# jizongFox/Self-paced-Contrastive-Learning

Hardware: AMD Instinct MI355X
Metric: pretrain slices/sec/node (UNet+InfoNCE, 224^2, bs=32/GPU) (higher is better)
Workload: dtype bf16; 1 GPU; BASELINE.json configs[1]: self-paced pretrain step, UNet base (max_channel=256) encoder to Conv5 + ProjectionHead(256,256,256) + SelfPacedSupConLoss(soft, partition labels, correct_grad) fwd+bwd + RAdam; slices_per_gpu=32, images_per_gpu_step=64, image=1x224x224, global_batch=32, parallelism=dp1, params=1311056, hipgraph=epocher, capture_steps=3

## Files before the change

include/spcl_hip.h:

```cpp
#ifndef SPCL_HIP_H
#define SPCL_HIP_H
#include <stddef.h>
#include <stdint.h>
#ifdef __cplusplus
extern "C" {
#endif

#define SPCL_F32 0
#define SPCL_BF16 1

#define SPCL_OK 0
#define SPCL_EINVAL (-1)
#define SPCL_ELAUNCH (-2)
#define SPCL_EUNSUPPORTED (-3)

#define SPCL_ABI_VERSION 18
int spcl_abi_version(void);
const char* spcl_last_error(void);

size_t spcl_supcon_workspace_bytes(int n, int d);
int spcl_supcon_forward(const float* z1, const float* z2, const float* labels, const float* mask, int n, int d,
                        float temperature, int sp_mode, float gamma, int correct_grad, float* ws, float* out,
                        void* stream);
int spcl_supcon_backward(const float* labels, const float* mask, int n, int d, float temperature, int sp_mode,
                         float gamma, const float* ws_fwd, float* ws_bwd, const float* out_fwd,
                         const float* grad_out, float* dz1, float* dz2, void* stream);
size_t spcl_supcon_bwd_workspace_bytes(int n, int d);
int spcl_supcon_unit_gradient_block(int n, int d, size_t* offset_floats, int* row_pitch);
int spcl_supcon_forward_heads(int K, const float* z1, const float* z2, size_t z_stride, const float* labels, int n,
                              int d, float temperature, int sp_mode, const float* gammas, int correct_grad, float* ws,
                              size_t ws_stride, float* out, void* stream);
int spcl_supcon_rows_supported(int n, int d);
int spcl_supcon_forward_rows(int K, const float* o1, const float* o2, size_t o_stride, const float* labels, int n, int d,
                             float temperature, int sp_mode, const float* gammas, int correct_grad, float* ws,
                             size_t ws_stride, float* out, void* stream);
int spcl_supcon_backward_heads(int K, const float* labels, int n, int d, float temperature, int sp_mode,
                               const float* gammas, const float* ws_fwd, size_t ws_stride, float* ws_bwd,
                               size_t wsb_stride, const float* out_fwd, const float* grad_out, float* dz1, float* dz2,
                               size_t z_stride, void* stream);
int spcl_supcon_materialize(const float* labels, const float* mask, int n, int d, float temperature, int sp_mode,
                            float gamma, const float* ws_fwd, float* sim_logits, float* sim_exp, float* pos_mask,
                            float* neg_mask, float* sp_mask, void* stream);

size_t spcl_supcon_xpos_workspace_bytes(int n, int d);
int spcl_supcon_xpos_forward(const float* z1, const float* z2, const float* labels, const float* mask, int n, int d,
                             float temperature, float* ws, float* out, void* stream);
int spcl_supcon_xpos_backward(const float* z1, const float* z2, int n, int d, float temperature, const float* ws,
                              const float* grad_out, float* dz1, float* dz2, void* stream);

// ... 28 lines not shown

int spcl_conv_pack_weights_block(const float* wa_oihw, int CinA, int CoutA, void* a_fwd, void* a_dgrad,
                                 const float* wb_oihw, int CinB, int CoutB, void* b_fwd, void* b_dgrad, int dtype,
                                 void* stream);
int spcl_conv_pack_weights_block_at(const float* wa_oihw, int CinA, int CoutA, void* a_fwd, void* a_dgrad,
                                    const float* wb_oihw, int CinB, int CoutB, void* b_fwd, void* b_dgrad, int dtype,
                                    int H, int W, void* stream);

#define SPCL_PACK_MULTI_MAX 24
typedef struct spcl_pack_item {
  const float* w_oihw;
  void* fwd;
  void* dgrad;
  int Cin, Cout, H, W;
} spcl_pack_item;
int spcl_conv_pack_weights_multi(const spcl_pack_item* items, int n, int dtype, void* stream);
int spcl_conv_pack_weights_multi_acorr(const spcl_pack_item* items, int n, int dtype, const float* image, int N, int H,
                                       int W, float* acorr, void* stream);
int spcl_conv_pack_weights_multi_zero(const spcl_pack_item* items, int n, int dtype, const float* image, int N, int H, int W,
                                      float* acorr, void* zero, size_t zero_bytes, void* stream);

int spcl_conv_num_tiles(int N, int H, int W);
int spcl_conv_stat_rows(int dtype, int N, int H, int W, int CinK, int CoutS);
void spcl_conv_set_gemm(int mode);
void spcl_conv_set_f32_split(int on);
int spcl_conv_get_f32_split(void);
size_t spcl_bn_stats_elems(int ntiles, int CS);
int spcl_conv3x3_forward(const void* x, int dtype, int N, int H, int W, int CinS, int CinK, int CoutS,
                         const void* w_packed, int in_mode, const float* in_scale, const float* in_shift, void* y,
                         float* stats, void* stream);
int spcl_conv3x3_forward_image_acorr_rows(int dtype, int N, int H, int W, int CinS, int CoutS);
int spcl_conv3x3_forward_image_acorr(const void* x, int dtype, int N, int H, int W, int CinS, int CoutS,
                                     const void* w_packed, void* y, float* stats, float* acorr_rows, void* stream);
int spcl_conv_cat_supported(int dtype, int N, int H, int W, int Chalf, int CoutS);
int spcl_conv3x3_forward_cat(const void* xa, const void* xb, int dtype, int N, int H, int W, int Chalf, int CoutS,
                             const void* w_packed, const float* xb_scale, const float* xb_shift, void* y, float* stats,
                             void* stream);
int spcl_conv3x3_wgrad_cat(const void* xa, const void* xb, const void* dy, int dtype, int N, int H, int W, int Chalf,
                           int Cout, int CoutS, const float* xb_scale, const float* xb_shift, float* partial,
                           float* dw_oihw, void* stream);
int spcl_conv_up2_supported(int dtype, int N, int H, int W, int CinK, int CoutS);
int spcl_conv3x3_forward_up2(const void* x_half, int dtype, int N, int H, int W, int CinK, int CoutS, const void* w_packed,
                             void* y, float* stats, void* stream);
int spcl_conv3x3_wgrad_up2(const void* x_half, const void* dy, int dtype, int N, int H, int W, int Cin, int Cout, int CoutS,
                           float* partial, float* dw_oihw, void* stream);
int spcl_conv_split_supported(int dtype, int N, int H, int W, int CinK, int CoutS);
int spcl_conv3x3_forward_split(const void* x, int dtype, int N, int H, int W, int CinK, int CoutS, const void* w_packed,
                               void* y_lo, void* y_hi, void* stream);
int spcl_conv_split_bnstats_supported(int dtype, int N, int H, int W, int CinK, int CoutS);
int spcl_conv3x3_dgrad_split_bnstats(const void* dy, int dtype, int N, int H, int W, int CinK, int CoutS,
                                     const void* w_packed, void* g_lo, void* g_hi, const void* y2_hi, const float* scale2,
                                     const float* shift2, const float* mean2, float* rows2, void* stream);

size_t spcl_conv_wgrad_workspace_bytes(int N, int H, int W, int CinK, int CoutS);
int spcl_conv3x3_wgrad(const void* x, const void* dy, int dtype, int N, int H, int W, int Cin, int CinS, int CinK,
                       int Cout, int CoutS, int in_mode, const float* in_scale, const float* in_shift, float* partial,
                       float* dw_oihw, void* stream);

int spcl_adaptive_pool2d_forward(const void* x, int dtype, int N, int H, int W, int C, int Cs, int OH, int OW, int mode,
                                 float* out, int* argmax, void* stream);
int spcl_adaptive_pool2d_backward(const float* dout, const int* argmax, int dtype, int N, int H, int W, int C, int Cs,
                                  int OH, int OW, int mode, void* dx, void* stream);

int spcl_l2norm_rows_forward(const float* x, size_t rows, int O, float* z, void* stream);
int spcl_l2norm_rows_backward(const float* x, const float* dz, size_t rows, int O, float* dx, void* stream);

// ... 57 lines not shown
                                      const float* scale, const float* shift, int training, float* ws, float* dgamma,
                                      float* dbeta, void* dy, void* stream);
int spcl_bnrelu_backward_up2(const void* y, const void* d_up, void* dact, int dtype, int N, int H, int W, int C, int CS,
                             const float* mean, const float* invstd, const float* scale, const float* shift, int training,
                             float* ws, float* dgamma, float* dbeta, void* dy, void* stream);
int spcl_bnrelu_backward_bcast(const void* y, const void* dact_nc, int dtype, int N, int H, int W, int C, int CS,
                               const float* mean, const float* invstd, const float* scale, const float* shift, int training,
                               float* ws, float* dgamma, float* dbeta, void* dy, void* stream);

size_t spcl_bnrelu_image_wgrad_workspace_bytes(int N, int H, int W, int CS);
int spcl_bnrelu_backward_image_wgrad(const void* y, const void* dact, const float* image, int dtype, int N, int H,
                                     int W, int C, int CS, const float* mean, const float* invstd, const float* scale,
                                     const float* shift, int training, float* ws, float* dgamma, float* dbeta,
                                     float* dw, void* stream);

int spcl_conv_dgrad_bnstats_supported(int dtype, int N, int H, int W, int CinK, int CoutS);
int spcl_conv3x3_dgrad_bnstats(const void* dy, int dtype, int N, int H, int W, int CinK, int CoutS, const void* w_packed,
                               void* g, const void* y2, const float* scale2, const float* shift2, const float* mean2,
                               float* rows2, void* stream);

int spcl_image_autocorr_rows(int N, int H, int W);
int spcl_image_autocorr(const float* image, int N, int H, int W, float* out, void* stream);
int spcl_conv_dgrad_bnstats_image_supported(int dtype, int N, int H, int W, int CinK, int CoutS);
int spcl_conv3x3_dgrad_bnstats_image(const void* dy, int dtype, int N, int H, int W, int CinK, int CoutS,
                                     const void* w_packed, void* g, const void* y2, const float* scale2,
                                     const float* shift2, const float* mean2, const float* image, float* rows11,
                                     void* stream);
int spcl_conv16_bwd_fused_supported(int dtype, int N, int H, int W, int CinK, int CoutS);
int spcl_conv16_bwd_fused_splits(int N, int H, int W);
int spcl_conv16_bwd_fused(const void* dy, int dtype, int N, int H, int W, const void* w_packed_dgrad, const void* y2,
                          const float* scale2, const float* shift2, const float* mean2, const float* image,
                          float* rows11, float* partial, float* dw_oihw, int Cin, int Cout, float* wg_rows,
                          const float* acorr, int nacorr, float* acorr16, void* stream);
int spcl_bnrelu_backward_wgrows_image3(const float* wg_rows, int nwg, const float* acorr, int nacorr, const float* w_oihw,
                                       int N, int H, int W, int C, int CS, const float* mean, const float* invstd,
                                       const float* scale, int training, float* ws, float* dgamma, float* dbeta,
                                       float* dw, void* stream);
size_t spcl_bnrelu_image3_workspace_bytes(int CS);
int spcl_bnrelu_backward_rows_image3(const float* rows11, int nrows, const float* acorr, int nacorr, const float* w_oihw,
                                     int N, int H, int W, int C, int CS, const float* mean, const float* invstd,
                                     const float* scale, int training, float* ws, float* dgamma, float* dbeta, float* dw,
                                     void* stream);

int spcl_conv_dgrad_poolstats_supported(int dtype, int N, int H, int W, int CinK, int CoutS, int H2, int W2);
int spcl_conv3x3_dgrad_poolstats(const void* dy, int dtype, int N, int H, int W, int CinK, int CoutS, const void* w_packed,
                                 void* g, const void* y2, int H2, int W2, const float* scale2, const float* shift2,
                                 const float* mean2, float* rows2, void* stream);
int spcl_bnrelu_pool_backward_rows(const void* y, const void* dpool, const float* rows, int nrows, int dtype, int N, int H,
                                   int W, int C, int CS, const float* mean, const float* invstd, const float* scale,
                                   const float* shift, int training, float* ws, float* dgamma, float* dbeta, void* dy,
                                   void* stream);
int spcl_bnrelu_backward_rows(const void* y, const void* dact, const float* image, const float* rows, int nrows, int dtype,
                              int N, int H, int W, int C, int CS, const float* mean, const float* invstd,
                              const float* scale, const float* shift, int training, float* ws, float* dgamma,
                              float* dbeta, void* dy, float* dw, void* stream);


int spcl_conv1x1_forward(const void* x, int dtype, size_t npix, int C, int CS, int K, const float* w, const float* b,
                         float* out, void* stream);
size_t spcl_conv1x1_bwd_workspace_bytes(int C, int K);
int spcl_conv1x1_backward(const void* x, const float* dout, int dtype, size_t npix, int C, int CS, int K, const float* w,
                          void* dx, float* dw, float* db, float* ws, void* stream);
int spcl_conv1x1_forward_bn(const void* y, int dtype, size_t npix, int C, int CS, int K, const float* scale,
                            const float* shift, const float* w, const float* b, float* out, void* stream);
int spcl_conv1x1_bwd_rows(size_t npix);
int spcl_conv1x1_backward_bn(const void* y, const float* dout, int dtype, size_t npix, int C, int CS, int K,
// ... 203 lines not shown
```

self-paced-contrastive-learning_amd/csrc/conv.hip:

```cpp
#include <stdlib.h>
#include "bn_acc.hpp"
#include "conv_common.hpp"
#include "image_acorr.hpp"

namespace spcl {

#ifndef SPCL_SPLIT_KC_MAX
#define SPCL_SPLIT_KC_MAX 64
#endif
__host__ __device__ inline int split_kc(int CinK, int CoutS) {
  const int cap = CoutS <= 16 ? 16 : (CoutS <= 32 ? 32 : SPCL_SPLIT_KC_MAX);
  return CinK < cap ? CinK : cap;
}
__host__ __device__ inline int split_pstride(int KC) {
  const int b = 3 * KC * 2;
  return (b / 32) % 2 == 1 ? b : b + 32;
}
__device__ __forceinline__ f32x4 mfma_bf16(u32x4 w, u32x4 x, f32x4 acc) {
  return __builtin_amdgcn_mfma_f32_16x16x32_bf16(__builtin_bit_cast(bf16x8, w), __builtin_bit_cast(bf16x8, x), acc, 0, 0, 0);
}

template <typename T, int TH, int TW, int NT, bool SPLIT = false>
__global__ __launch_bounds__(256) void conv3x3_mfma_kernel(ConvArgs a) {
  static_assert(!SPLIT || sizeof(T) == 4, "the split k-loop is the f32 storage path");
// ... 1062 lines not shown
  else if (dtype == SPCL_BF16) rc = launch_conv_t<bf16_t>(a, st);
  else {
    set_error("conv3x3_forward: dtype %d", dtype);
    return SPCL_EINVAL;
  }
  if (rc != 0) {
    set_error("conv3x3_forward: no kernel for N=%d H=%d W=%d CinK=%d CoutS=%d in_mode=%d", N, H, W, CinK, CoutS, in_mode);
    return SPCL_EUNSUPPORTED;
  }
  SPCL_LAUNCH_CHECK("conv3x3_forward");
  return SPCL_OK;
}

static bool image_acorr_args(ConvArgs& a, int dtype, int N, int H, int W, int CinS, int CoutS) {
  static const bool off = lab_env("SPCL_ACORR_IN_CONV", 1) == 0;
  if (off || dtype != SPCL_BF16 || N <= 0 || H <= 0 || W <= 0 || CinS != 1 || CoutS != 16) return false;
  a.N = N; a.H = H; a.W = W; a.CinS = CinS; a.CinK = 16; a.CoutS = CoutS; a.in_mode = 2;
  a.tilesX = a.tilesY = 0; a.tpw = 1; a.dbg = 0;
  const TileCfg t = pick_tile_k(H, W, 16, CoutS);
  static const int no_fast = lab_env("SPCL_CONV_NO_FAST", 0);
  return !no_fast && t.tw == 14 && t.th == 14 && H % 14 == 0 && W % 14 == 0;
}

extern "C" int spcl_conv3x3_forward_image_acorr_rows(int dtype, int N, int H, int W, int CinS, int CoutS) {
  ConvArgs a;
  float dummy = 0.f;
  a.x = nullptr; a.y = nullptr; a.wp = nullptr; a.stats = nullptr; a.in_scale = a.in_shift = nullptr;
  if (!image_acorr_args(a, dtype, N, H, W, CinS, CoutS)) return 0;
  a.acorr_rows = &dummy;
  if (!launch_conv_fast(a, 14, nullptr, true)) return 0;
  return N * cdiv(H, 14) * cdiv(W, 14);
}

extern "C" int spcl_conv3x3_forward_image_acorr(const void* x, int dtype, int N, int H, int W, int CinS, int CoutS,
                                                const void* w_packed, void* y, float* stats, float* acorr_rows,
                                                void* stream) {
  SPCL_CHECK_ARG(x && y && w_packed && acorr_rows, "conv3x3_forward_image_acorr: null pointer");
  ConvArgs a;
  a.x = x; a.y = y; a.wp = w_packed; a.stats = stats; a.in_scale = a.in_shift = nullptr;
  if (!image_acorr_args(a, dtype, N, H, W, CinS, CoutS)) {
    set_error("conv3x3_forward_image_acorr: unsupported configuration (ask spcl_conv3x3_forward_image_acorr_rows)");
    return SPCL_EUNSUPPORTED;
  }
  a.acorr_rows = acorr_rows;
  {
    const double px = (double)N * H * W;
    prof_cost(px * (4.0 + CoutS * 2.0) + 9.0 * 16 * CoutS * 2.0 + (double)N * cdiv(H, 14) * cdiv(W, 14) * 256.0,
              2.0 * px * 9.0 * CinS * CoutS + 2.0 * px * 2.0 * 256.0);
  }
  if (!launch_conv_fast(a, 14, (hipStream_t)stream)) {
    set_error("conv3x3_forward_image_acorr: no kernel for N=%d H=%d W=%d", N, H, W);
    return SPCL_EUNSUPPORTED;
  }
  SPCL_LAUNCH_CHECK("conv3x3_forward_image_acorr");
  return SPCL_OK;
}

static bool conv_cat_args(ConvArgs& a, int dtype, int N, int H, int W, int Chalf, int CoutS) {
  static const bool off = lab_env("SPCL_CONV_CAT", 1) == 0;
  if (off || dtype != SPCL_BF16 || N <= 0 || H <= 0 || W <= 0 || CoutS % 16 != 0 || CoutS <= 0 ||
      (Chalf != 16 && Chalf != 32 && Chalf != 64 && Chalf != 128))
    return false;
  if ((2 * Chalf) % 64 == 0 && CoutS % 64 == 0 && Chalf % 64 != 0) return false;
  a.in_scale = a.in_shift = nullptr;
  a.stats = nullptr;
  a.N = N; a.H = H; a.W = W; a.CinS = 2 * Chalf; a.CinK = 2 * Chalf; a.CoutS = CoutS; a.in_mode = 0;
  a.tilesX = a.tilesY = 0;
  a.tpw = 1;
  a.dbg = 0;
  return !conv_use_gemm(a.CinK, CoutS, H, W) && pick_tile(H, W).tw == 14;
}

extern "C" int spcl_conv_cat_supported(int dtype, int N, int H, int W, int Chalf, int CoutS) {
  ConvArgs a;
  if (!conv_cat_args(a, dtype, N, H, W, Chalf, CoutS)) return 0;
  static const char dummy[16] = {0};
  a.x = dummy; a.x2 = dummy; a.y = nullptr; a.wp = nullptr;
  return launch_conv_fast(a, pick_tile_k(H, W, a.CinK).th, nullptr, true) ? 1 : 0;
}

extern "C" int spcl_conv3x3_forward_cat(const void* xa, const void* xb, int dtype, int N, int H, int W, int Chalf, int CoutS,
                                        const void* w_packed, const float* xb_scale, const float* xb_shift, void* y,
                                        float* stats, void* stream) {
  SPCL_CHECK_ARG(xa && xb && y && w_packed, "conv3x3_forward_cat: null pointer");
  SPCL_CHECK_ARG((xb_scale == nullptr) == (xb_shift == nullptr), "conv3x3_forward_cat: xb_scale and xb_shift come together");
  SPCL_CHECK_ARG(xb_scale == nullptr || Chalf <= 32, "conv3x3_forward_cat: the raw second tensor exists for Chalf 16 / 32 only");
  SPCL_CHECK_ARG((uintptr_t)xa % 16 == 0 && (uintptr_t)xb % 16 == 0, "conv3x3_forward_cat: inputs must be 16-byte aligned");
// ... 343 lines not shown
```

self-paced-contrastive-learning_amd/csrc/conv16_bwd.hip:

```cpp
#include <stdio.h>
#include <stdlib.h>
#include <vector>
#include "conv_common.hpp"

namespace spcl {

struct Bwd16Args {
  const unsigned char* dy;
  const u32x4* wp;
  const unsigned char* y2;
  const float* scale2;
  const float* shift2;
  const float* mean2;
  const float* img;
  float* rows11;
  float* wg_rows;
  int nwg;
  const float* acorr_in;
  int nacorr;
  float* acorr_out;
  float* partial;
  int N, H, W, tilesX, tilesY, ipw, xcd_remap;
  int dbg;
  unsigned long long* stamps;
};

constexpr int B16_TH = 14, B16_TW = 14, B16_HW = 16, B16_RP = 22, B16_PS = 32;
constexpr int B16_DY = 0, B16_DY_BYTES = (B16_TH + 2) * B16_RP * B16_PS;
constexpr int B16_IM = B16_DY_BYTES, B16_IM_BYTES = 1536;
constexpr int B16_XT = B16_IM + B16_IM_BYTES, B16_XT_ROW = 16 * 32, B16_XT_BYTES = B16_TH * B16_XT_ROW;
constexpr int B16_RED = B16_XT + B16_XT_BYTES;
constexpr int B16_ACC = B16_RED + 512;
constexpr int B16_TRASH = B16_ACC + 576;
constexpr int B16_LDS = B16_TRASH + 32;

#ifndef SPCL_CONV16_DBG_BUILD
#define SPCL_CONV16_DBG_BUILD 0
#endif
#define B16_DBG(a) (SPCL_CONV16_DBG_BUILD ? (a).dbg : 0)

__device__ __forceinline__ bf16x8 b16_tr_frag(unsigned addr) {
  const s16x4 lo = __builtin_amdgcn_ds_read_tr16_b64_v4i16((s16x4 __attribute__((address_space(3)))*)(uintptr_t)addr);
  const s16x4 hi =
// ... 360 lines not shown
        for (int w = 1; w < NW; ++w) tot += red[32 * w];
      } else {
        tot = ((const float*)(lds + B16_ACC))[i - 32];
      }
      a.wg_rows[(size_t)i * a.nwg + wg] = tot;
    }
  }
  float* out = a.partial + wg * (9 * 256);
#pragma unroll
  for (int j = 0; j < TPW; ++j) {
    const int tap = wave + NW * j;
    if (tap < 9) {
#pragma unroll
      for (int r = 0; r < 4; ++r) out[(tap * 16 + 4 * ((t0 & 63) >> 4) + r) * 16 + (t0 & 15)] = wacc[j][r];
    }
  }
}


#ifndef SPCL_CONV16_ROWS_WPE
#define SPCL_CONV16_ROWS_WPE 4
#endif
constexpr int r16_wpe(bool shifted) { return shifted && SPCL_CONV16_ROWS_WPE > 3 ? 3 : SPCL_CONV16_ROWS_WPE; }
constexpr int R16_RP = 18;
constexpr int R16_DY = 0, R16_DY_BYTES = (B16_TH + 2) * R16_RP * B16_PS;
constexpr int R16_IM = R16_DY_BYTES;
constexpr int R16_XT = R16_IM + B16_IM_BYTES;
constexpr int R16_RED = R16_XT + B16_XT_BYTES;
constexpr int R16_ACC = R16_RED + 512;
constexpr int R16_TRASH = R16_ACC + 576;
constexpr int R16_TAB = R16_TRASH + 32;
constexpr int B16_LDS_ROWS = R16_TAB + 128;

template <bool SHIFTED, bool WGROWS>
__global__ __launch_bounds__(128) __attribute__((amdgpu_waves_per_eu(r16_wpe(SHIFTED)))) void conv16_bwd_rows_kernel(Bwd16Args a) {
  constexpr int NW = 2;
  constexpr int TH = B16_TH, TW = B16_TW, HW_ = B16_HW, RP = R16_RP, PS = B16_PS;
  constexpr int NSTEPS = 5, NTHR = 64 * NW, ITER = 512 / NTHR, RPI = NTHR / 32;
  constexpr int MW = TH / NW, TPW = (9 + NW - 1) / NW;
  static_assert(TH % NW == 0, "rows are dealt to the waves evenly");
  extern __shared__ __attribute__((aligned(16))) unsigned char lds[];
  const unsigned lds_base = (unsigned)(uintptr_t)(unsigned char __attribute__((address_space(3)))*)lds;
  const int t0 = threadIdx.x;
  const int wave = __builtin_amdgcn_readfirstlane(t0 >> 6);
  if (WGROWS && (int)blockIdx.z * (int)(gridDim.x * gridDim.y) >= a.nwg) {
    const int nslice = gridDim.x * gridDim.y;
    float* fold = (float*)lds;
    const int cq = t0 & 15, rl = t0 >> 4;
    for (int j = blockIdx.y * gridDim.x + blockIdx.x; j < 16; j += nslice) {
      f32x4 sacc = {0.f, 0.f, 0.f, 0.f};
#pragma unroll 16
      for (int w = j + 16 * rl; w < a.nacorr; w += 128) sacc += *(const f32x4*)(a.acorr_in + (size_t)w * 64 + 4 * cq);
      __syncthreads();
      *(f32x4*)(fold + rl * 64 + 4 * cq) = sacc;
      __syncthreads();
      if (t0 < 64) {
        float tot = fold[t0];
#pragma unroll
        for (int r = 1; r < 8; ++r) tot += fold[r * 64 + t0];
        a.acorr_out[(size_t)j * 64 + t0] = tot;
      }
    }
    return;
  }

  int tx = blockIdx.x, ty = blockIdx.y;
  {
    const int T = a.tilesX * a.tilesY;
// ... 1 lines not shown
      const int L = ty * a.tilesX + tx;
      const int L2 = (L & 7) * (T >> 3) + (L >> 3);
      ty = L2 / a.tilesX;
      tx = L2 - ty * a.tilesX;
    }
  }
  const int y0 = min(ty * TH, a.H - TH), x0 = min(tx * TW, a.W - TW);
  const int oy = ty * TH - y0, ox = tx * TW - x0;
  const bool interior = y0 > 0 && x0 > 0 && y0 + TH < a.H && x0 + TW < a.W;
  const bool shifted = SHIFTED && (oy | ox) != 0;

  if (t0 < 4 * TH) *(u32x4*)(lds + R16_XT + (t0 >> 2) * B16_XT_ROW + TW * PS + (t0 & 3) * 16) = (u32x4){0u, 0u, 0u, 0u};
  if (t0 >= NTHR - 64)
    *(u32x4*)(lds + R16_DY + (((t0 & 63) >> 2) * RP + HW_) * PS + (t0 & 3) * 16) = (u32x4){0u, 0u, 0u, 0u};
  if (t0 < 48) {
    const int r = t0 & 15, k = t0 >> 4;
    ((bf16_t*)(lds + R16_IM))[(k == 0 ? 256 + 15 : (k == 1 ? 512 + 14 : 512 + 15)) + r * 16] = 0;
  }
  if (t0 >= 64 && t0 < 64 + 20) {
    const int e = t0 - 64, gq = e / NSTEPS, s = e - gq * NSTEPS;
    int fc = 4 * s + gq;
    if (fc >= 18) fc = 0;
    const int tap = fc >> 1, c = fc & 1, ky = (tap * 11) >> 5, kx = tap - 3 * ky;
    ((unsigned*)(lds + R16_TAB))[gq * 8 + s] = (unsigned)((ky * RP + kx) * PS + c * 16);
  }
  if (WGROWS)
    for (int i = t0; i < (512 + 576) / 4; i += NTHR) ((float*)(lds + R16_RED))[i] = 0.f;
  f32x4 wacc[TPW];
#pragma unroll
  for (int j = 0; j < TPW; ++j) wacc[j] = (f32x4){0.f, 0.f, 0.f, 0.f};

  float imgv[256 / NTHR];
  u32x4 v[ITER];
  uint2 ypre[MW];
  constexpr int PPT = 256 / NTHR;
  auto rsrc = [](const void* p) { return __builtin_amdgcn_make_buffer_rsrc((void*)p, 0, 0x7fffffff, 0x00020000); };
  constexpr int OOB = (int)0x80000000u;
  auto issue_img = [&](const int n) {
    int t = t0;
    asm volatile("" : "+v"(t));
    const int hr = (t * PPT) >> 4, hc = (t * PPT) & 15;
    const int gy = y0 - 1 + hr;
    const __amdgpu_buffer_rsrc_t rs = rsrc(a.img + (size_t)n * a.H * a.W);
    const int rowo = (gy < 0 ? 0 : (gy >= a.H ? a.H - 1 : gy)) * a.W;
#pragma unroll
    for (int e = 0; e < PPT; ++e) {
      const int gx = x0 - 1 + hc + e;
      imgv[e] = __builtin_bit_cast(float, __builtin_amdgcn_raw_buffer_load_b32(rs, (rowo + (gx < 0 ? 0 : (gx >= a.W ? a.W - 1 : gx))) * 4, 0, 0));
    }
  };
  auto issue_halo = [&](const int n) {
    int t = t0;
    asm volatile("" : "+v"(t));
    const int ch = t & 1, q0 = t >> 1, hy0 = q0 / HW_, hx0 = q0 % HW_;
    const int voff = (hy0 * a.W + hx0) * 32 + ch * 16;
    const __amdgpu_buffer_rsrc_t rs = rsrc(a.dy + (((long)n * a.H + (y0 - 1)) * a.W + (x0 - 1)) * 32);
#pragma unroll
    for (int k = 0; k < ITER; ++k) {
      bool inb = true;
      if (!interior) {
        const int gy = y0 - 1 + hy0 + RPI * k, gx = x0 - 1 + hx0;
        inb = gy >= 0 && gy < a.H && gx >= 0 && gx < a.W;
      }
      v[k] = __builtin_bit_cast(u32x4, __builtin_amdgcn_raw_buffer_load_b128(rs, inb ? voff : OOB, RPI * k * a.W * 32, 0));
    }
  };
  auto issue_y2 = [&](const int n) {
    int t = t0;
    asm volatile("" : "+v"(t));
    const int r16 = t & 15, g = (t & 63) >> 4;
    const int voff = min(r16, TW - 1) * 32 + g * 8;
    const __amdgpu_buffer_rsrc_t rs = rsrc(a.y2 + (((size_t)n * a.H + y0 + wave) * a.W + x0) * 32);
#pragma unroll
    for (int j = 0; j < MW; ++j)
      ypre[j] = __builtin_bit_cast(uint2, __builtin_amdgcn_raw_buffer_load_b64(rs, voff, NW * j * a.W * 32, 0));
  };
  const __amdgpu_buffer_rsrc_t rs_wp = rsrc(a.wp), rs_sc = rsrc(a.scale2), rs_sh = rsrc(a.shift2), rs_mu = rsrc(a.mean2);

  const bool stamp = SPCL_CONV16_STAMPS_BUILD && a.stamps != nullptr && t0 == 0;
  unsigned long long tph[7] = {0, 0, 0, 0, 0, 0, 0}, tc = 0;
  const int n_first = blockIdx.z * a.ipw;
  if (stamp) tc = __builtin_amdgcn_s_memtime();
  if (n_first < a.N) {
    issue_img(n_first);
    issue_halo(n_first);
    issue_y2(n_first);
  }
  __syncthreads();
  uint2 dzp[MW];
  auto second_half = [&](const int n) {
    int t = t0;
    asm volatile("" : "+v"(t));
    const int lane = t & 63, r16 = t & 15, g = lane >> 4;
    const int tile = (n * a.tilesY + ty) * a.tilesX + tx;
    const unsigned xaddr = (unsigned)(R16_XT + wave * B16_XT_ROW + r16 * PS + (((g + (r16 >> 2)) & 3) << 3));
    B16_STAMP(3)
    __syncthreads();
    B16_STAMP(1)
    if (!WGROWS && t < 32) {
      const float* red = (const float*)(lds + R16_RED) + t;
      float tot = red[0];
#pragma unroll
      for (int w = 1; w < NW; ++w) tot += red[32 * w];
      a.rows11[(size_t)tile * 11 * 16 + t] = tot;
    }

    const unsigned tr_col = (unsigned)((4 * (g & 1) + (r16 >> 2)) * PS + (r16 & 3) * 8);
    const unsigned tr_x = lds_base + R16_XT + (g >> 1) * B16_XT_ROW + (4 * (g & 1) + (r16 >> 2)) * PS + ((((r16 & 3) + (g & 1)) & 3) << 3);
    const unsigned tr_xh = (tr_x + 8 * PS) ^ 16u;
    {
      unsigned ad[TPW];
#pragma unroll
      for (int j = 0; j < TPW; ++j) {
        const int tap = min(wave + NW * j, 8), ky = tap / 3, kx = tap - 3 * ky;
        ad[j] = lds_base + R16_DY + (g >> 1) * RP * PS + tr_col + (2 - ky) * RP * PS + (2 - kx) * PS;
      }
#pragma unroll
      for (int ks = 0; ks < TH / 2; ++ks) {
        const bf16x8 af = b16_tr_frag2(tr_x + ks * 2 * B16_XT_ROW, tr_xh + ks * 2 * B16_XT_ROW);
// ... 49 lines not shown
    const f32x4 mu2 = __builtin_bit_cast(f32x4, __builtin_amdgcn_raw_buffer_load_b128(rs_mu, g * 16, 0, 0));
    if (r16 >= TW || (SHIFTED && r16 < ox)) {
      sc2 = (f32x4){0.f, 0.f, 0.f, 0.f};
      sh2 = (f32x4){-1.f, -1.f, -1.f, -1.f};
    }
    const u32x4 tabA = *(const u32x4*)(lds + R16_TAB + g * 32);
    const unsigned tabB = *(const unsigned*)(lds + R16_TAB + g * 32 + 16);
    {
      const int hr = (t * PPT) >> 4, hc = (t * PPT) & 15;
      const int gy = y0 - 1 + hr;
#pragma unroll
      for (int e = 0; e < PPT; ++e) {
        const int gx = x0 - 1 + hc + e;
        const float hv = (interior || (gy >= 0 && gy < a.H && gx >= 0 && gx < a.W)) ? imgv[e] : 0.f;
        const bf16_t hb = f32_to_bf16(hv);
        bf16_t* imb = (bf16_t*)(lds + R16_IM) + hr * 16 + hc + e;
        imb[0] = hb;
        if (hc + e >= 1) imb[256 - 1] = hb;
        if (hc + e >= 2) imb[512 - 2] = hb;
      }
    }
    {
      const int ch = t & 1, q0 = t >> 1, hy0 = q0 / HW_, hx0 = q0 % HW_;
      unsigned char* const lp = lds + R16_DY + (hy0 * RP + hx0) * PS + ch * 16;
#pragma unroll
      for (int k = 0; k < ITER; ++k) *(u32x4*)(lp + (RPI * k * RP) * PS) = v[k];
    }
    B16_STAMP(0)
    __syncthreads();
    B16_STAMP(1)

    f32x4 ssum = {0.f, 0.f, 0.f, 0.f}, ssq = {0.f, 0.f, 0.f, 0.f};
    const unsigned xaddr = (unsigned)(R16_XT + wave * B16_XT_ROW + r16 * PS + (((g + (r16 >> 2)) & 3) << 3));
    {
      const unsigned lb = (unsigned)(R16_DY + (wave * RP + r16) * PS);
      const unsigned offs[NSTEPS] = {tabA[0] + lb, tabA[1] + lb, tabA[2] + lb, tabA[3] + lb, tabB + lb};
#pragma unroll
      for (int j = 0; j < MW; ++j) {
        f32x4 acc = {0.f, 0.f, 0.f, 0.f};
#pragma unroll
        for (int s = 0; s < NSTEPS; ++s) {
          const u32x4 xf = *(const u32x4*)(lds + offs[s] + j * (NW * RP * PS));
          acc = mfma_chunk<bf16_t>(wall[s], xf, acc);
        }
        const bool keep_y = !shifted || wave + NW * j >= oy;
        const float yv[4] = {__uint_as_float(ypre[j].x << 16), __uint_as_float(ypre[j].x & 0xffff0000u),
                             __uint_as_float(ypre[j].y << 16), __uint_as_float(ypre[j].y & 0xffff0000u)};
        const f32x2 glo = {acc[0], acc[1]}, ghi = {acc[2], acc[3]};
        const uint32_t g0 = __builtin_bit_cast(uint32_t, __builtin_convertvector(glo, bf16x2v));
        const uint32_t g1 = __builtin_bit_cast(uint32_t, __builtin_convertvector(ghi, bf16x2v));
        const float gv[4] = {__uint_as_float(g0 << 16), __uint_as_float(g0 & 0xffff0000u),
                             __uint_as_float(g1 << 16), __uint_as_float(g1 & 0xffff0000u)};
        float xv[4], dz[4];
#pragma unroll
        for (int r = 0; r < 4; ++r) {
          float z = fmaf(sc2[r], yv[r], sh2[r]);
          if (SHIFTED) z = keep_y ? z : -1.f;
          xv[r] = z;
          dz[r] = z > 0.f ? gv[r] : 0.f;
          ssum[r] += dz[r];
          ssq[r] = fmaf(dz[r], yv[r] - mu2[r], ssq[r]);
        }
        const f32x2 lo = {xv[0], xv[1]}, hi = {xv[2], xv[3]};
        uint2 w;
        w.x = relu_bf16x2(__builtin_bit_cast(uint32_t, __builtin_convertvector(lo, bf16x2v)));
        w.y = relu_bf16x2(__builtin_bit_cast(uint32_t, __builtin_convertvector(hi, bf16x2v)));
        *(uint2*)(lds + xaddr + j * (NW * B16_XT_ROW)) = w;
        dzp[j].x = (__float_as_uint(dz[0]) >> 16) | (__float_as_uint(dz[1]) & 0xffff0000u);
        dzp[j].y = (__float_as_uint(dz[2]) >> 16) | (__float_as_uint(dz[3]) & 0xffff0000u);
        asm volatile("" : "+v"(dzp[j].x), "+v"(dzp[j].y));
        __builtin_amdgcn_sched_barrier(0);
      }
    }
    B16_STAMP(2)
    {
      f32x4 o;
#pragma unroll
      for (int r = 0; r < 4; ++r) {
        const float s1 = row16_sum(ssum[r]), s2 = row16_sum(ssq[r]);
        o[r] = r16 == 0 ? s1 : s2;
      }
      if (r16 < 2) {
        f32x4* rp = (f32x4*)(lds + R16_RED + ((wave * 2 + r16) * 16 + 4 * g) * 4);
        *rp = WGROWS ? *rp + o : o;
      }
    }
    if (!(it + 1 < a.ipw && n + 1 < a.N)) break;
    issue_halo(n + 1);
    issue_y2(n + 1);
    issue_img(n + 1);
    second_half(n);
  }
  if (n_first < a.N) second_half(n);

  if (stamp) {
    unsigned long long* o = a.stamps + ((size_t)(blockIdx.z * gridDim.y + blockIdx.y) * gridDim.x + blockIdx.x) * 8;
#pragma unroll
    for (int k = 0; k < 7; ++k) o[k] = tph[k];
  }
  const size_t wg = (size_t)(blockIdx.z * gridDim.y + blockIdx.y) * gridDim.x + blockIdx.x;
  if (WGROWS) {
    __syncthreads();
    for (int i = t0; i < 11 * 16; i += NTHR) {
      float tot;
      if (i < 32) {
        const float* red = (const float*)(lds + R16_RED) + i;
        tot = red[0];
#pragma unroll
        for (int w = 1; w < NW; ++w) tot += red[32 * w];
      } else {
        tot = ((const float*)(lds + R16_ACC))[i - 32];
      }
      a.wg_rows[(size_t)i * a.nwg + wg] = tot;
    }
  }
  float* out = a.partial + wg * (9 * 256);
#pragma unroll
  for (int j = 0; j < TPW; ++j) {
    const int tap = wave + NW * j;
    if (tap < 9) {
#pragma unroll
      for (int r = 0; r < 4; ++r) out[(tap * 16 + 4 * ((t0 & 63) >> 4) + r) * 16 + (t0 & 15)] = wacc[j][r];
// ... 8 lines not shown

int conv16_bwd_nw() {
  static const int env = lab_env("SPCL_CONV16_NW", 2);
  return env == 1 || env == 4 ? env : 2;
}

int conv16_bwd_ipw(int N, int H, int W) {
  const int nw = conv16_bwd_nw();
  const int resident = 256 * (nw == 1 ? 8 : (nw == 2 ? (conv16_bwd_rowmap() ? 2 * SPCL_CONV16_ROWS_WPE : 6) : 3));
  const long tiles = (long)cdiv(H, B16_TH) * cdiv(W, B16_TW);
  static const int env_ipw = lab_env("SPCL_CONV16_IPW", 0);
  int ipw = env_ipw > 0 ? env_ipw : (int)((tiles * N + resident - 1) / resident);
  if (ipw < 1) ipw = 1;
  if (ipw > N) ipw = N;
  return ipw;
}

}

using namespace spcl;

extern "C" int spcl_conv16_bwd_fused_supported(int dtype, int N, int H, int W, int CinK, int CoutS) {
  static const bool off = lab_flag("SPCL_NO_CONV16_FUSED");
  if (off || CinK != 16 || CoutS != 16) return 0;
  return spcl_conv_dgrad_bnstats_image_supported(dtype, N, H, W, CinK, CoutS);
}

extern "C" int spcl_conv16_bwd_fused_splits(int N, int H, int W) {
  if (N <= 0 || H < B16_TH || W < B16_TW) return 0;
  const int ipw = conv16_bwd_ipw(N, H, W);
  return cdiv(H, B16_TH) * cdiv(W, B16_TW) * cdiv(N, ipw);
}

extern "C" int spcl_conv16_bwd_fused(const void* dy, int dtype, int N, int H, int W, const void* w_packed_dgrad,
                                     const void* y2, const float* scale2, const float* shift2, const float* mean2,
                                     const float* image, float* rows11, float* partial, float* dw_oihw, int Cin, int Cout,
                                     float* wg_rows, const float* acorr, int nacorr, float* acorr16, void* stream) {
  SPCL_CHECK_ARG(dy && w_packed_dgrad && y2 && scale2 && shift2 && mean2 && image && partial && dw_oihw,
                 "conv16_bwd_fused: null pointer");
  SPCL_CHECK_ARG((rows11 != nullptr) != (wg_rows != nullptr), "conv16_bwd_fused: exactly one of rows11 / wg_rows");
  SPCL_CHECK_ARG(wg_rows == nullptr || (acorr && acorr16 && nacorr > 0), "conv16_bwd_fused: wg_rows comes with the autocorrelation rows");
  SPCL_CHECK_ARG(Cin > 0 && Cin <= 16 && Cout > 0 && Cout <= 16, "conv16_bwd_fused: channel counts");
  if (!spcl_conv16_bwd_fused_supported(dtype, N, H, W, 16, 16)) {
    set_error("conv16_bwd_fused: unsupported configuration (bf16, 16 -> 16 channels, 14 x 14 tiles)");
    return SPCL_EUNSUPPORTED;
  }
  hipStream_t st = (hipStream_t)stream;
  spcl_wgrad_tail* tail = take_tail_capture();
  Bwd16Args a;
  a.dy = (const unsigned char*)dy; a.wp = (const u32x4*)w_packed_dgrad; a.y2 = (const unsigned char*)y2;
  a.scale2 = scale2; a.shift2 = shift2; a.mean2 = mean2; a.img = image; a.rows11 = rows11; a.partial = partial;
  a.wg_rows = wg_rows; a.acorr_in = acorr; a.nacorr = nacorr; a.acorr_out = acorr16;
  a.N = N; a.H = H; a.W = W; a.tilesX = cdiv(W, B16_TW); a.tilesY = cdiv(H, B16_TH);
  a.ipw = conv16_bwd_ipw(N, H, W);
  static const int env_remap = lab_env("SPCL_CONV_XCD_REMAP", 1);
  a.xcd_remap = env_remap;
  a.dbg = lab_env("SPCL_CONV16_DBG", 0);
  const int nz = cdiv(N, a.ipw), nsplit = a.tilesX * a.tilesY * nz;
  a.nwg = nsplit;
  const double px = (double)N * H * W;
  prof_cost(px * 32.0 * 2.0 + px * 4.0 + (double)nsplit * 9 * 256 * 4.0, 2.0 * px * 9.0 * 256 * 2.0 + 2.0 * px * 9.0 * 16);
  a.stamps = nullptr;
  const bool want_stamps = SPCL_CONV16_STAMPS_BUILD && lab_flag("SPCL_CONV16_STAMPS");
  const size_t nwg = (size_t)nsplit;
  if (want_stamps) {
    (void)hipMalloc(&a.stamps, nwg * 8 * sizeof(unsigned long long));
    (void)hipMemset(a.stamps, 0, nwg * 8 * sizeof(unsigned long long));
  }
  const int nw = conv16_bwd_nw();
  const bool even = H % B16_TH == 0 && W % B16_TW == 0, wgr = wg_rows != nullptr;
  const dim3 grid(a.tilesX, a.tilesY, nz + (wgr ? 1 : 0));
#define B16_LAUNCH(SH_, NW_, WG_) SPCL_LAUNCH((conv16_bwd_kernel<SH_, NW_, WG_>), grid, dim3(64 * NW_), B16_LDS, st, a)
#define B16_CASE(NW_)                                       \
  if (nw == NW_) {                                          \
    if (even && wgr) B16_LAUNCH(false, NW_, true);          \
    else if (even) B16_LAUNCH(false, NW_, false);           \
    else if (wgr) B16_LAUNCH(true, NW_, true);              \
    else B16_LAUNCH(true, NW_, false);                      \
  }
  if (nw == 2 && conv16_bwd_rowmap()) {
#define B16_ROWS(SH_, WG_) SPCL_LAUNCH((conv16_bwd_rows_kernel<SH_, WG_>), grid, dim3(128), B16_LDS_ROWS, st, a)
    if (even && wgr) B16_ROWS(false, true);
    else if (even) B16_ROWS(false, false);
    else if (wgr) B16_ROWS(true, true);
    else B16_ROWS(true, false);
#undef B16_ROWS
  }
#if SPCL_LAB
  else {
    B16_CASE(1) B16_CASE(2) B16_CASE(4)
  }
#endif
#undef B16_CASE
#undef B16_LAUNCH
  if (a.stamps != nullptr) {
    std::vector<unsigned long long> h(nwg * 8);
    (void)hipStreamSynchronize(st);
    (void)hipMemcpy(h.data(), a.stamps, h.size() * 8, hipMemcpyDeviceToHost);
    (void)hipFree(a.stamps);
    double ph[7] = {0, 0, 0, 0, 0, 0, 0};
    for (size_t i = 0; i < nwg; ++i)
      for (int k = 0; k < 7; ++k) ph[k] += (double)h[i * 8 + k];
    fprintf(stderr, "[conv16_bwd stamps] %zu workgroups x %d tiles | s_memtime ticks of wave 0 per TILE: staging %.0f, barriers %.0f, "
            "dgrad %.0f, pixel pass %.0f, wgrad %.0f, dz stores %.0f, tap sums %.0f\n", nwg, a.ipw, ph[0] / nwg / a.ipw,
            ph[1] / nwg / a.ipw, ph[2] / nwg / a.ipw, ph[3] / nwg / a.ipw, ph[4] / nwg / a.ipw, ph[5] / nwg / a.ipw,
            ph[6] / nwg / a.ipw);
  }
  if (tail != nullptr) {
    tail->partial = partial; tail->dw = dw_oihw; tail->kind = 0; tail->nsplit = nsplit; tail->nblk_ci = 1;
    tail->nblk_co = 1; tail->CIB = 16; tail->COB = 16; tail->Cin = Cin; tail->Cout = Cout;
  } else {
    launch_wgrad_reduce(partial, nsplit, 1, 1, 16, 16, Cin, Cout, dw_oihw, st);
  }
  SPCL_LAUNCH_CHECK("conv16_bwd_fused");
  return SPCL_OK;
}
```

self-paced-contrastive-learning_amd/csrc/conv_common.hpp:

```cpp
#pragma once
#include "common.hpp"

namespace spcl {

struct BnAccFwd;
template <typename T> struct Chunk;
template <> struct Chunk<float> { static constexpr int EPC = 4; };
template <> struct Chunk<bf16_t> { static constexpr int EPC = 8; };

struct uint4_ { uint32_t x, y, z, w; };
typedef __attribute__((ext_vector_type(4))) uint32_t u32x4;

__host__ __device__ inline int conv_kc(int CinK) { return CinK < 64 ? CinK : 64; }
template <typename T> __host__ __device__ inline int conv_pstride(int KC) {
  int b = KC * (int)sizeof(T);
  return b == 32 ? 32 : b + 32;
}
template <typename T> __host__ __device__ inline int conv_nsteps(int KC) {
  int cp = KC / Chunk<T>::EPC;
  return (9 * cp + 3) / 4;
}

struct ConvArgs {
  const void* x;
  void* y;
  const void* wp;
  float* stats;
  const float* in_scale;
  const float* in_shift;
  int N, H, W;
  int CinS;
  int CinK;
  int CoutS;
  int in_mode;
  int tilesX, tilesY;
  int tpw;
  int dbg;
  const void* y2 = nullptr;
  const float* scale2 = nullptr;
  const float* shift2 = nullptr;
  const float* mean2 = nullptr;
  float* rows2 = nullptr;
  int H2 = 0, W2 = 0;
  const float* img2 = nullptr;
  const void* x2 = nullptr;
  void* y_hi = nullptr;
  bool x_up2 = false;
  float* acorr_rows = nullptr;
  long long* stats_acc = nullptr;
  long long* rows2_acc = nullptr;
  const struct BnAccFwd* in_bn = nullptr;
};

struct split_f32 { float v; };
template <> struct Chunk<split_f32> { static constexpr int EPC = 4; };
bool conv_f32_split();

typedef __attribute__((ext_vector_type(2))) float f32x2_;
typedef __attribute__((ext_vector_type(2))) __bf16 bf16x2v_;
struct Split3 { uint32_t hi, mid, lo; };
__device__ __forceinline__ Split3 split3_pair(float v0, float v1) {
  Split3 o;
  f32x2_ v = {v0, v1};
  o.hi = __builtin_bit_cast(uint32_t, __builtin_convertvector(v, bf16x2v_));
  v[0] -= __uint_as_float(o.hi << 16);
  v[1] -= __uint_as_float(o.hi & 0xffff0000u);
  o.mid = __builtin_bit_cast(uint32_t, __builtin_convertvector(v, bf16x2v_));
  v[0] -= __uint_as_float(o.mid << 16);
  v[1] -= __uint_as_float(o.mid & 0xffff0000u);
  o.lo = __builtin_bit_cast(uint32_t, __builtin_convertvector(v, bf16x2v_));
  return o;
}
__device__ __forceinline__ void split3_chunk(const float* e, u32x4& ph, u32x4& pm, u32x4& pl) {
#pragma unroll
  for (int k = 0; k < 4; ++k) {
    const Split3 o = split3_pair(e[2 * k], e[2 * k + 1]);
    ph[k] = o.hi;
    pm[k] = o.mid;
    pl[k] = o.lo;
  }
}
// ... 90 lines not shown
```

self-paced-contrastive-learning_amd/csrc/conv_fast.hip:

```cpp
#include <stdlib.h>
#include <type_traits>
#include <vector>
#include "bn_acc.hpp"
#include "conv_common.hpp"

namespace spcl {

struct FastArgs {
  const unsigned char* x;
  const unsigned char* x2;
  unsigned char* y;
  unsigned char* y_hi;
  int up2;
  const u32x4* wp;
  float* stats;
  const float* in_scale;
  const float* in_shift;
  int N, H, W, CinK, CoutS, tilesX, tilesY, gy;
  unsigned long long* stamps;
  int lds_flip;
  int xcd_remap;
  const unsigned char* y2;
  const float* scale2;
  const float* shift2;
  const float* mean2;
  float* rows2;
  int H2, W2;
  const float* img2;
  float* acorr_rows;
  long long* stats_acc;
  long long* rows2_acc;
  BnAccFwd in_bn;
};

#ifndef SPCL_FAST_WPE_NT1
#define SPCL_FAST_WPE_NT1 2
#endif
#ifndef SPCL_FAST_WPE_NT1_NW4
#define SPCL_FAST_WPE_NT1_NW4 3
#endif
#ifndef SPCL_FAST_WR_NT1
#define SPCL_FAST_WR_NT1 9
#endif
#ifndef SPCL_FAST_WPE_KC32
#define SPCL_FAST_WPE_KC32 2
#endif
#ifndef SPCL_FAST_YPRE_MINKC
#define SPCL_FAST_YPRE_MINKC 16
#endif
#ifndef SPCL_FAST_WIDE_STORES
#define SPCL_FAST_WIDE_STORES 1
#endif
#ifndef SPCL_FAST_DBG
#define SPCL_FAST_DBG 0
#endif
#ifndef SPCL_FAST_ROWMAP
#define SPCL_FAST_ROWMAP 1
#endif
#ifndef SPCL_FAST_RP
#define SPCL_FAST_RP (SPCL_FAST_ROWMAP ? 18 : 22)
#endif
#ifndef SPCL_FAST_RP_NARROW
#define SPCL_FAST_RP_NARROW (SPCL_FAST_ROWMAP ? 18 : 22)
#endif
constexpr int fast_pixel_stride(int KC) { return KC == 16 ? 32 : KC * 2 + 32; }
constexpr int fast_row_pitch(int KC) { return KC == 64 ? SPCL_FAST_RP : SPCL_FAST_RP_NARROW; }
constexpr int fast_lds_bytes(int KC, int TH) { return (TH + 2) * fast_row_pitch(KC) * fast_pixel_stride(KC); }
constexpr bool fast_preload_slab(int KC, int NW, int NT) { return KC == 32 || (KC == 64 && NW >= 2 && NT >= 1); }
constexpr int fast_wpe(int KC, int TH, int NW, int NT, int MODE = 0) {
  const int wgs = 160 * 1024 / fast_lds_bytes(KC, TH);
  int w = (wgs * NW + 3) / 4;
  w = w > 4 ? 4 : (w < 1 ? 1 : w);
  const int acc = (SPCL_FAST_ROWMAP ? TH : (TH * 14 + 15) / 16) * NT * 4;
  if (KC == 16 && MODE >= 2 && SPCL_FAST_YPRE_MINKC <= 16 && w > 3 && acc <= 80) return 3;
  if (acc > 80 && w > 2) return 2;
  if (KC == 64 && NT == 1 && NW == 4 && w > 2) return SPCL_FAST_WPE_NT1_NW4;
  if (KC == 64 && NT == 1 && NW >= 2 && w > 2) return SPCL_FAST_WPE_NT1;
  if (KC == 32 && fast_preload_slab(KC, NW, NT) && w > SPCL_FAST_WPE_KC32) return SPCL_FAST_WPE_KC32;
  if (fast_preload_slab(KC, NW, NT) && w > 2) return 2;
  return w;
}

template <int KC, int TH, int NT, int MODE, int NW>
__global__ __launch_bounds__(64 * NW) __attribute__((amdgpu_waves_per_eu(fast_wpe(KC, TH, NW, NT, MODE)))) void
conv3x3_fast_kernel(FastArgs a) {
  constexpr int TW = 14, HW_ = 16, CP = KC / 8, NHALO = (TH + 2) * HW_, PS = fast_pixel_stride(KC);
  constexpr int RP = fast_row_pitch(KC);
  constexpr int NTHR = 64 * NW, NCH = NHALO * CP, ITER = (NCH + NTHR - 1) / NTHR, QS = NTHR / CP;
  constexpr bool RM = SPCL_FAST_ROWMAP != 0;
  constexpr int NPIX = TH * TW, MT = RM ? TH : (NPIX + 15) / 16, NSTEPS = (9 * CP + 3) / 4;
  constexpr bool PRELOAD_W = KC == 16;
  constexpr bool PRELOAD_SLAB = fast_preload_slab(KC, NW, NT);
  static_assert(QS >= HW_ ? QS % HW_ == 0 : HW_ % QS == 0, "staging walk needs whole/even halo rows per iteration");
  extern __shared__ __attribute__((aligned(16))) unsigned char lds[];

  const int t = threadIdx.x, lane = t & 63, wave = t >> 6, r16 = lane & 15, g = lane >> 4;
#ifndef SPCL_FAST_STAMPS_BUILD
#define SPCL_FAST_STAMPS_BUILD 0
#endif
  const bool stamp = SPCL_FAST_STAMPS_BUILD && a.stamps != nullptr && t == 0;
  unsigned long long t_begin = 0, t_k0 = 0, t_k1 = 0, t_store = 0;
  if (stamp) t_begin = __builtin_amdgcn_s_memtime();
  int tx = blockIdx.x, ty = blockIdx.y;
  {
    const int T = a.tilesX * a.tilesY;
    if (a.xcd_remap && (T & 7) == 0) {
      const int L = ty * a.tilesX + tx;
      const int L2 = (L & 7) * (T >> 3) + (L >> 3);
      ty = L2 / a.tilesX;
      tx = L2 - ty * a.tilesX;
    }
  }
  int n = blockIdx.z, by = 0;
#if SPCL_FAST_DBG & 4
  if (KC == 64 && a.CinK >= 128 && gridDim.z == 2u * a.N * a.gy) n >>= 1;
#endif
  if (a.gy > 1) {
    by = n / a.N;
    n -= by * a.N;
  }
  const int y0 = min(ty * TH, a.H - TH), x0 = min(tx * TW, a.W - TW);
  const int oy = ty * TH - y0, ox = tx * TW - x0;
  const int tile = (n * a.tilesY + ty) * a.tilesX + tx;
  const int ntn = a.CoutS >> 4;
  const int nt0 = (by * NW + wave) * NT;
  const bool interior = y0 > 0 && x0 > 0 && y0 + TH < a.H && x0 + TW < a.W;
#if SPCL_FAST_DBG & 4
  const int nslab = KC < 64 ? 1 : ((a.CinK >= 128 && gridDim.z == 2u * a.N * a.gy) ? a.CinK / KC / 2 : a.CinK / KC);
#else
  const int nslab = KC < 64 ? 1 : a.CinK / KC;
#endif
  const int gps = (KC < 64 ? KC : a.CinK) * 2;

  constexpr bool M2 = MODE == 2 || MODE == 4;
  constexpr bool M1 = MODE == 1 || MODE >= 5;
  constexpr int ACC_TPC = MODE == 5 ? 4 : (MODE == 6 ? 2 : 1);
  float imgv[MODE == 4 ? 4 : 1];
  if (MODE == 4) {
    const int hr = lane >> 2, hc = (lane & 3) * 4;
    const int gy = y0 - 1 + hr;
    const float* ir = a.img2 + ((size_t)n * a.H + (gy < 0 ? 0 : (gy >= a.H ? a.H - 1 : gy))) * a.W;
#pragma unroll
    for (int e = 0; e < 4; ++e) {
      const int gx = x0 - 1 + hc + e;
      const bool in = gy >= 0 && gy < a.H && gx >= 0 && gx < a.W;
      const float xv = ir[gx < 0 ? 0 : (gx >= a.W ? a.W - 1 : gx)];
      imgv[e] = in ? xv : 0.f;
    }
  }

  u32x4 wall[PRELOAD_W ? NSTEPS : 1][NT];
  if (PRELOAD_W) {
#pragma unroll
    for (int s = 0; s < NSTEPS; ++s)
#pragma unroll
      for (int j = 0; j < NT; ++j) wall[s][j] = a.wp[(size_t)(s * ntn + nt0 + j) * 64 + lane];
  }

  const int ch = t & (CP - 1), q0 = t / CP;
  const int hy0 = q0 / HW_, hx0 = q0 % HW_;
  const bool two = a.x2 != nullptr;
  const bool two_chunks = two && a.CinK == KC;
  const int gps1 = two ? gps / 2 : gps;
  const int ch1 = two_chunks ? (ch & (CP / 2 - 1)) : ch;
  const long xorg = (((long)n * a.H + (y0 - 1)) * a.W + (x0 - 1)) * gps1;
  const unsigned char* xb = ((two_chunks && ch >= CP / 2) ? a.x2 : a.x) + xorg;
  const unsigned char* xb2 = two ? a.x2 + xorg : nullptr;
  const unsigned voff = (unsigned)((hy0 * a.W + hx0) * gps1 + ch1 * 16);
  unsigned char* const lp = lds + (hy0 * RP + hx0) * PS + ch * 16;

  int abase[MT];
#pragma unroll
  for (int i = 0; i < MT; ++i) {
    if (RM) {
      abase[i] = (i * RP + r16) * PS + (CP >= 4 ? g * 16 : 0);
    } else {
      int p = 16 * i + r16;
      if (p >= NPIX) p = 0;
      const int py = p / TW, px = p - py * TW;
      abase[i] = (py * RP + px) * PS + (CP >= 4 ? g * 16 : 0);
    }
  }
  f32x4 acc[MT][NT];
#pragma unroll
  for (int i = 0; i < MT; ++i)
#pragma unroll
    for (int j = 0; j < NT; ++j) acc[i][j] = (f32x4){0.f, 0.f, 0.f, 0.f};

  const int flip = a.lds_flip;
  const unsigned wvo = (unsigned)(nt0 * 64 + lane) * 16u;
  const size_t wstep = (size_t)ntn * 1024;
  u32x4 v[ITER];
  float ssc[8], ssh[8];
  constexpr bool STREAM_W = PRELOAD_SLAB && KC == 64;
  constexpr int WR = STREAM_W ? (NT == 1 ? SPCL_FAST_WR_NT1 : 9) : (PRELOAD_SLAB ? NSTEPS : 1);
  u32x4 wsl[WR][NT];
  constexpr bool acc_in = MODE >= 5;
  float* const coef_l = (float*)(lds + fast_lds_bytes(KC, TH) * (a.lds_flip != 0 ? 2 : 1));
  auto load_coef_lds = [&](int slab) {
    const int cc = two_chunks ? ch1 : ch;
#pragma unroll
    for (int e = 0; e < 8; e += 4) {
      *(f32x4*)&ssc[e] = *(const f32x4*)(coef_l + slab * KC + cc * 8 + e);
      *(f32x4*)&ssh[e] = *(const f32x4*)(coef_l + a.CinK + slab * KC + cc * 8 + e);
    }
  };
  auto issue_halo = [&](int slab, const bool first = false) {
    if (acc_in) {
      if (!first) load_coef_lds(slab);
    } else if (M1) {
#pragma unroll
      for (int e = 0; e < 8; e += 4) {
        const int cc = two_chunks ? ch1 : ch;
        *(f32x4*)&ssc[e] = *(const f32x4*)(a.in_scale + slab * KC + cc * 8 + e);
        *(f32x4*)&ssh[e] = *(const f32x4*)(a.in_shift + slab * KC + cc * 8 + e);
      }
    }
    const int hslab = (a.CinK / KC) >> 1;
    const unsigned char* xs = (two && !two_chunks) ? (slab >= hslab ? xb2 + (slab - hslab) * (KC * 2) : xb + slab * (KC * 2))
                                                   : xb + slab * (KC * 2);
    auto walk = [&](auto up2_c, auto interior_c) {
      constexpr bool UP2 = decltype(up2_c)::value, INTERIOR = decltype(interior_c)::value;
#pragma unroll
      for (int k = 0; k < ITER; ++k) {
        const int dky = QS >= HW_ ? k * (QS / HW_) : k / (HW_ / QS);
        const int dkx = QS >= HW_ ? 0 : (k % (HW_ / QS)) * QS;
        const long soff = ((long)dky * a.W + dkx) * gps1;
        bool inb = (NCH % NTHR == 0) || (k * NTHR + t < NCH);
        if (!INTERIOR) {
          const int gy = y0 - 1 + hy0 + dky, gx = x0 - 1 + hx0 + dkx;
// ... 3 lines not shown
        if (UP2) {
          const int gy = y0 - 1 + hy0 + dky, gx = x0 - 1 + hx0 + dkx;
          if (inb)
            v[k] = *(const u32x4*)(a.x + (((long)n * (a.H >> 1) + (gy >> 1)) * (a.W >> 1) + (gx >> 1)) * gps + slab * (KC * 2) +
                                   ch * 16);
        } else if (inb) v[k] = *(const u32x4*)(xs + soff + voff);
      }
    };
    if (a.up2) walk(std::true_type{}, std::false_type{});
    else if (interior) walk(std::false_type{}, std::true_type{});
    else walk(std::false_type{}, std::false_type{});
  };
  unsigned char* lpw = lp;
  auto slab_body = [&](const int slab, const bool refill) {
    auto stage = [&](auto interior_c) {
      constexpr bool INTERIOR = decltype(interior_c)::value;
#pragma unroll
      for (int k = 0; k < ITER; ++k) {
        const int dky = QS >= HW_ ? k * (QS / HW_) : k / (HW_ / QS);
        const int dkx = QS >= HW_ ? 0 : (k % (HW_ / QS)) * QS;
        const bool in_range = (NCH % NTHR == 0) || (k * NTHR + t < NCH);
        u32x4 tv = v[k];
        if (M1) {
          bool inb = true;
          if (!INTERIOR) {
            const int gy = y0 - 1 + hy0 + dky, gx = x0 - 1 + hx0 + dkx;
            inb = gy >= 0 && gy < a.H && gx >= 0 && gx < a.W;
          }
          if (inb && (!two_chunks || ch >= CP / 2)) tv = bnrelu_regs<bf16_t>(tv, ssc, ssh);
        }
        if (in_range) *(u32x4*)(lpw + (dky * RP + dkx) * PS) = tv;
      }
    };
    if (M1 && !interior) stage(std::false_type{});
    else stage(std::true_type{});
    if (refill) issue_halo(slab + 1);
    if (stamp && slab == 0) t_store = __builtin_amdgcn_s_memtime();
    __syncthreads();
    if (stamp && slab == 0) t_k0 = __builtin_amdgcn_s_memtime();

    const u32x4* wslab = a.wp + ((size_t)slab * NSTEPS * ntn + nt0) * 64 + lane;
    auto frag_off = [&](const int s) {
      if (CP >= 4) {
        const int fc0 = 4 * s, tap = fc0 / CP, c0 = fc0 % CP, ky = tap / 3, kx = tap % 3;
        return (ky * RP + kx) * PS + c0 * 16;
      }
      int fc = 4 * s + g;
      if (fc >= 9 * CP) fc = 0;
      const int tap = fc / CP, c = fc % CP, ky = (tap * 11) >> 5, kx = tap - 3 * ky;
      return (ky * RP + kx) * PS + c * 16;
    };
    if (STREAM_W) {
      const __amdgpu_buffer_rsrc_t wrs = __builtin_amdgcn_make_buffer_rsrc((void*)a.wp, 0, 0x7fffffff, 0x00020000);
      unsigned wrun = (unsigned)(((size_t)slab * NSTEPS + WR) * wstep);
      u32x4 xf[2][MT];
#pragma unroll
      for (int i = 0; i < MT; ++i) xf[0][i] = *(const u32x4*)(lds + abase[i] + frag_off(0));
#pragma unroll
      for (int s = 0; s < NSTEPS; ++s) {
        u32x4 wf[NT];
#pragma unroll
        for (int j = 0; j < NT; ++j) wf[j] = wsl[s % WR][j];
#pragma unroll
        for (int i = 0; i < MT; ++i) {
#pragma unroll
          for (int j = 0; j < NT; ++j) acc[i][j] = mfma_chunk<bf16_t>(wf[j], xf[s & 1][i], acc[i][j]);
          if (s + 1 < NSTEPS && !(SPCL_FAST_DBG & 2)) xf[(s + 1) & 1][i] = *(const u32x4*)(lds + abase[i] + frag_off(s + 1));
// ... 6 lines not shown
        }
        wrun += (unsigned)wstep;
      }
    } else {
#pragma unroll
      for (int s = 0; s < NSTEPS; ++s) {
        u32x4 wf[NT];
#pragma unroll
        for (int j = 0; j < NT; ++j)
          wf[j] = PRELOAD_W ? wall[s][j] : (PRELOAD_SLAB ? wsl[s][j] : wslab[(size_t)(s * ntn + j) * 64]);
        const int off = frag_off(s);
#pragma unroll
        for (int i = 0; i < MT; ++i) {
          const u32x4 xf = *(const u32x4*)(lds + abase[i] + off);
#pragma unroll
          for (int j = 0; j < NT; ++j) acc[i][j] = mfma_chunk<bf16_t>(wf[j], xf, acc[i][j]);
          if (RM && !PRELOAD_SLAB && i % 7 == 6) __builtin_amdgcn_sched_barrier(0);
        }
      }
    }
  };
#ifndef SPCL_ACC_DBG
#define SPCL_ACC_DBG 0
#endif
  const int acc_part = acc_in ? t / a.CinK : 0, acc_c = t - acc_part * a.CinK;
  constexpr int ACC_RPT = BN_ACC_REPLICAS / ACC_TPC > 0 ? BN_ACC_REPLICAS / ACC_TPC : 1;
  const bool acc_has = acc_part * ACC_RPT < BN_ACC_REPLICAS;
  BnAccPart<ACC_RPT> accp;
  BnAccFwdParams accprm;
  if (acc_in && SPCL_ACC_DBG < 2) {
    accp.load(a.in_bn.acc, a.CinK, acc_c, acc_has ? ACC_RPT * acc_part : 0);
    accprm.load(a.in_bn, acc_c);
  }
  issue_halo(0, true);
  if (PRELOAD_SLAB) {
#pragma unroll
    for (int s = 0; s < WR; ++s)
#pragma unroll
      for (int j = 0; j < NT; ++j) wsl[s][j] = a.wp[((size_t)s * ntn + nt0 + j) * 64 + lane];
  }
  if (acc_in) {
    const bool writer = (blockIdx.x | blockIdx.y | blockIdx.z) == 0;
    BnAccSums sums{0, 0, 0, 0, 0};
    if (SPCL_ACC_DBG < 2 && acc_has) sums = accp.sums();
    if (SPCL_ACC_DBG < 2) sums.flag = accp.flag;
    if (ACC_TPC > 1) {
      long long* const part_l = (long long*)(coef_l + 2 * a.CinK);
      if (acc_part > 0) {
        long long* q = part_l + ((size_t)(acc_part - 1) * a.CinK + acc_c) * 4;
        *(i64x2*)q = (i64x2){sums.h1, sums.l1};
        *(i64x2*)(q + 2) = (i64x2){sums.h2, sums.l2};
      }
      __syncthreads();
      if (acc_part == 0) {
#pragma unroll
        for (int k = 1; k < ACC_TPC; ++k) {
          const long long* q = part_l + ((size_t)(k - 1) * a.CinK + acc_c) * 4;
          const i64x2 u = *(const i64x2*)q, w = *(const i64x2*)(q + 2);
          sums.h1 += u[0]; sums.l1 += u[1]; sums.h2 += w[0]; sums.l2 += w[1];
        }
      }
    }
    if (t < a.CinK) {
      float sc_, sh_;
      if (SPCL_ACC_DBG == 0) bn_acc_fwd_channel(a.in_bn, sums, accprm, t, sc_, sh_, writer);
      else { sc_ = a.in_bn.gamma[t]; sh_ = a.in_bn.beta[t]; }
      coef_l[t] = sc_;
// ... 263 lines not shown
      const unsigned char* pa = lds + M4_DZ + r16 * 448 + (g >> 1) * 32 + (g & 1) * 16;
      const unsigned char* pb = lds + M4_IM + tkx * 512 + ((g >> 1) + tky) * 32 + (g & 1) * 16;
      f32x4 D = {0.f, 0.f, 0.f, 0.f};
#pragma unroll
      for (int ks = 0; ks < TH / 2; ++ks)
        D = mfma_chunk<bf16_t>(*(const u32x4*)(pa + ks * 64), *(const u32x4*)(pb + ks * 64), D);
      if (r16 < 9) *(f32x4*)(a.rows2 + ((size_t)tile * RS + 2 + r16) * a.CoutS + nt0 * 16 + 4 * g) = D;
    }
  } else if ((MODE == 0 || M1) && a.stats_acc != nullptr) {
#pragma unroll
    for (int j = 0; j < NT; ++j) {
      f32x4 s1, s2;
#pragma unroll
      for (int r = 0; r < 4; ++r) {
        s1[r] = row16_sum(ssum[j][r]);
        s2[r] = row16_sum(ssq[j][r]);
      }
      bn_acc_add_row16(a.stats_acc, a.CoutS, replica, (nt0 + j) * 16 + 4 * g, r16, s1, s2);
    }
  } else if (a.stats != nullptr) {
#pragma unroll
    for (int j = 0; j < NT; ++j)
      write_tile_stats(a.stats, tile, a.CoutS, (nt0 + j) * 16 + 4 * g, r16, (float)((TH - oy) * (TW - ox)), ssum[j],
                       ssq[j]);
  }
  if (stamp) {
    __builtin_amdgcn_s_waitcnt(0);
    const unsigned long long t_end = __builtin_amdgcn_s_memtime();
    unsigned long long* o = a.stamps + ((size_t)(blockIdx.z * gridDim.y + blockIdx.y) * gridDim.x + blockIdx.x) * 4;
    o[0] = t_store - t_begin; o[1] = t_k0 - t_store; o[2] = t_k1 - t_k0; o[3] = t_end - t_k1;
  }
}

template <int TH, bool EVEN, bool ACORR = false>
__global__ __launch_bounds__(64) __attribute__((amdgpu_waves_per_eu(4))) void conv3x3_image_kernel(FastArgs a) {
  constexpr int TW = 14, HW_ = 16, LW = HW_ + 2;
  constexpr bool RM = SPCL_FAST_ROWMAP != 0;
  constexpr int NPIX = TH * TW, MT = RM ? TH : (NPIX + 15) / 16, NHALO = (TH + 2) * HW_;
  __shared__ uint32_t pairs[(TH + 2) * LW];
  const int lane = threadIdx.x, r16 = lane & 15, g = lane >> 4;
  int tx = blockIdx.x, ty = blockIdx.y;
  const int n = blockIdx.z;
  {
    const int T = a.tilesX * a.tilesY;
    if (a.xcd_remap && (T & 7) == 0) {
      const int L = ty * a.tilesX + tx;
      const int L2 = (L & 7) * (T >> 3) + (L >> 3);
      ty = L2 / a.tilesX;
      tx = L2 - ty * a.tilesX;
    }
  }
  const int y0 = min(ty * TH, a.H - TH), x0 = min(tx * TW, a.W - TW);
  const int oy = ty * TH - y0, ox = tx * TW - x0;
  const int tile = (n * a.tilesY + ty) * a.tilesX + tx;

  s16x4 wfrag = {0, 0, 0, 0};
  if (g < 3) {
    const bf16_t* wp = (const bf16_t*)a.wp;
#pragma unroll
    for (int kx = 0; kx < 3; ++kx) {
      const int tap = 3 * g + kx;
      wfrag[kx] = (short)wp[(size_t)(((tap >> 1) * 64) + (2 * (tap & 1)) * 16 + r16) * 8];
    }
  }

  const float* img = (const float*)a.x + (size_t)n * a.H * a.W;
  {
    const int hx = r16, gx = x0 - 1 + hx;
    const bool colok = gx >= 0 && gx < a.W;
    const int gxc = gx < 0 ? 0 : (gx >= a.W ? a.W - 1 : gx);
#pragma unroll
    for (int k = 0; k < (NHALO + 63) / 64; ++k) {
      const int hy = g + 4 * k;
      const int gy = y0 - 1 + hy;
      const int gyc = gy < 0 ? 0 : (gy >= a.H ? a.H - 1 : gy);
      const float raw = img[(size_t)gyc * a.W + gxc];
      const float v0 = (colok && gy >= 0 && gy < a.H) ? raw : 0.f;
      float v1 = __shfl_down(v0, 1, 64);
      if (hx == HW_ - 1) v1 = 0.f;
      const f32x2 pv = {v0, v1};
      if (NHALO % 64 == 0 || hy < TH + 2) pairs[hy * LW + hx] = __builtin_bit_cast(uint32_t, __builtin_convertvector(pv, bf16x2v));
    }
  }
  if (lane < 2 * (TH + 2)) pairs[(lane >> 1) * LW + HW_ + (lane & 1)] = 0u;
  __syncthreads();

  f32x4 acc[MT];
#pragma unroll
  for (int i = 0; i < MT; ++i) {
    int p = 16 * i + r16;
    if (p >= NPIX) p = 0;
    const int py = RM ? i : p / TW, px = RM ? r16 : p - py * TW;
    const int gg = g < 3 ? g : 0;
    const uint32_t* src = pairs + (py + gg) * LW + px;
    const uint32_t lo = src[0], hi = src[2];
    const uint2 xv = {lo, hi};
    acc[i] = __builtin_amdgcn_mfma_f32_16x16x16bf16_1k(wfrag, __builtin_bit_cast(s16x4, xv),
                                                       (f32x4){0.f, 0.f, 0.f, 0.f}, 0, 0, 0);
  }

  constexpr int DPY = RM ? 1 : 16 / TW, DPX = RM ? 0 : 16 % TW;
  const int rowb = a.CoutS * 2;
  unsigned char* yb = a.y + (((size_t)n * a.H + y0) * a.W + x0) * rowb + 4 * g * 2;
  int py = RM ? 0 : r16 / TW, px = r16 - py * TW;
  int ob = (py * a.W + px) * rowb;
  const int dob = (DPY * a.W + DPX) * rowb, wrapo = (a.W - TW) * rowb;
  f32x4 ssum = {0.f, 0.f, 0.f, 0.f}, ssq = {0.f, 0.f, 0.f, 0.f};
  const bool shifted = !EVEN && (oy | ox) != 0;
  int pyc = py;
  uint2 pk[MT];
  int obs[MT];
  if (!RM || r16 < TW) {
#pragma unroll
  for (int i = 0; i < MT; ++i) {
    const bool ok = RM || (16 * i + 15 < NPIX) || (16 * i + r16 < NPIX);
    obs[i] = ob;
    {
      const f32x2 lo = {acc[i][0], acc[i][1]}, hi = {acc[i][2], acc[i][3]};
      pk[i].x = __builtin_bit_cast(uint32_t, __builtin_convertvector(lo, bf16x2v));
      pk[i].y = __builtin_bit_cast(uint32_t, __builtin_convertvector(hi, bf16x2v));
    }
    if (ok) {
      if (EVEN) {
        ssum += acc[i];
        ssq += acc[i] * acc[i];
      } else {
        const float keep = (!shifted || (pyc >= oy && px >= ox)) ? 1.f : 0.f;
        const f32x4 av = acc[i] * keep;
        ssum += av;
        ssq += av * acc[i];
      }
    }
    px += DPX;
    pyc += DPY;
    ob += dob;
    if (!RM && px >= TW) {
      px -= TW;
      pyc += 1;
      ob += wrapo;
    }
  }
  constexpr int NPAIR = SPCL_FAST_WIDE_STORES ? (RM ? MT / 2 : (NPIX / 16) / 2) : 0;
#pragma unroll
  for (int p = 0; p < NPAIR; ++p) {
    const int i = 2 * p;
    const auto rx = __builtin_amdgcn_permlane16_swap(pk[i].x, pk[i + 1].x, false, false);
    const auto ry = __builtin_amdgcn_permlane16_swap(pk[i].y, pk[i + 1].y, false, false);
    const u32x4 v = {rx[0], ry[0], rx[1], ry[1]};
    *(u32x4*)(yb + ((g & 1) ? obs[i + 1] - 8 : obs[i])) = v;
  }
#pragma unroll
  for (int i = 2 * NPAIR; i < MT; ++i) {
    const bool ok = RM || (16 * i + 15 < NPIX) || (16 * i + r16 < NPIX);
    if (ok) *(uint2*)(yb + obs[i]) = pk[i];
  }
  }
  if (a.stats != nullptr)
    write_tile_stats(a.stats, tile, a.CoutS, 4 * g, r16, (float)((TH - oy) * (TW - ox)), ssum, ssq);
  if (ACORR) {
    static_assert(!ACORR || (EVEN && TH % 2 == 0), "autocorrelation rows: whole 14 x 14 tiles");
    __shared__ float dsum[2][16][16];
    const int tap = r16 < 9 ? r16 : 0, ky = tap / 3, kx = tap - 3 * ky;
    const uint32_t* src = pairs + ((g >> 1) + ky) * LW + 8 * (g & 1) + kx;
    const bool upper = (g & 1) != 0;
    const u32x4 ones = {0x3f803f80u, 0x3f803f80u, 0x3f803f80u, 0x3f803f80u};
    f32x4 D = {0.f, 0.f, 0.f, 0.f}, S = {0.f, 0.f, 0.f, 0.f};
#pragma unroll
    for (int ks = 0; ks < TH / 2; ++ks) {
      const uint32_t* q = src + ks * 2 * LW;
      const u32x4 fb = {q[0], q[2], q[4], q[6]};
      u32x4 fa = fb;
      fa[3] = upper ? 0u : fb[3];
      D = __builtin_amdgcn_mfma_f32_16x16x32_bf16(__builtin_bit_cast(bf16x8, fa), __builtin_bit_cast(bf16x8, fb), D, 0, 0, 0);
      S = __builtin_amdgcn_mfma_f32_16x16x32_bf16(__builtin_bit_cast(bf16x8, fa), __builtin_bit_cast(bf16x8, ones), S, 0, 0, 0);
    }
#pragma unroll
    for (int r = 0; r < 4; ++r) {
      dsum[0][4 * g + r][r16] = D[r];
      dsum[1][4 * g + r][r16] = S[r];
    }
    __syncthreads();
    const int k = lane;
    float v = 0.f;
    if (k < 45) {
      int ra = 0;
#pragma unroll
      for (int i = 1; i < 9; ++i) ra += k >= i * 9 - i * (i - 1) / 2 ? 1 : 0;
      const int cb = ra + (k - (ra * 9 - ra * (ra - 1) / 2));
      v = dsum[0][ra][cb];
    } else if (k < 54) {
      v = dsum[1][k - 45][0];
    }
    a.acorr_rows[(size_t)tile * 64 + k] = v;
  }
}

template <int KC, int TH, int NT, int NW>
static void launch_fast(const FastArgs& a, int mode, hipStream_t st) {
  static const int env_pipe = lab_env("SPCL_CONV_FAST_PIPE", 1);
  const bool pipe = env_pipe && KC == 64 && a.CinK > KC;
  FastArgs b = a;
  b.lds_flip = pipe ? fast_lds_bytes(KC, TH) : 0;
  const size_t lds = fast_lds_bytes(KC, TH) * (pipe ? 2 : 1) + (a.img2 != nullptr ? 1536 : 0) +
                     (a.in_bn.acc != nullptr ? (size_t)a.CinK * 8 + (size_t)64 * NW * 32 : 0);
  dim3 grid(a.tilesX, a.tilesY, a.N * a.gy), block(64 * NW);
#if SPCL_FAST_DBG & 4
  if (KC == 64 && a.CinK >= 128 && (long)a.tilesX * a.tilesY * a.N * a.gy <= 256) grid.z *= 2;
#endif
  static const bool env_stamps = SPCL_FAST_STAMPS_BUILD && lab_flag("SPCL_FAST_STAMPS");
  const size_t nwg = (size_t)grid.x * grid.y * grid.z;
  b.stamps = nullptr;
  if (env_stamps) {
    (void)hipMalloc(&b.stamps, nwg * 4 * sizeof(unsigned long long));
    (void)hipMemset(b.stamps, 0, nwg * 4 * sizeof(unsigned long long));
  }
  if (a.img2 != nullptr) {
    if constexpr (KC == 16 && TH == 14 && NT == 1 && NW == 1)
      SPCL_LAUNCH((conv3x3_fast_kernel<KC, TH, NT, 4, NW>), grid, block, lds, st, b);
  } else if (mode == 1 && a.in_bn.acc != nullptr) {
    if constexpr (KC == 64) {
      const int tpc = 64 * NW / a.CinK;
      if (tpc == 4) SPCL_LAUNCH((conv3x3_fast_kernel<KC, TH, NT, 5, NW>), grid, block, lds, st, b);
      else if (tpc == 2) SPCL_LAUNCH((conv3x3_fast_kernel<KC, TH, NT, 6, NW>), grid, block, lds, st, b);
      else SPCL_LAUNCH((conv3x3_fast_kernel<KC, TH, NT, 7, NW>), grid, block, lds, st, b);
    }
  } else if (mode == 1) SPCL_LAUNCH((conv3x3_fast_kernel<KC, TH, NT, 1, NW>), grid, block, lds, st, b);
  else if (a.rows2 != nullptr && a.H2 > 0) SPCL_LAUNCH((conv3x3_fast_kernel<KC, TH, NT, 3, NW>), grid, block, lds, st, b);
  else if (a.rows2 != nullptr) SPCL_LAUNCH((conv3x3_fast_kernel<KC, TH, NT, 2, NW>), grid, block, lds, st, b);
  else SPCL_LAUNCH((conv3x3_fast_kernel<KC, TH, NT, 0, NW>), grid, block, lds, st, b);
  if (b.stamps != nullptr) {
    std::vector<unsigned long long> h(nwg * 4);
    (void)hipStreamSynchronize(st);
    (void)hipMemcpy(h.data(), b.stamps, h.size() * 8, hipMemcpyDeviceToHost);
    (void)hipFree(b.stamps);
    double s4[4] = {0, 0, 0, 0};
    for (size_t i = 0; i < nwg; ++i)
      for (int k = 0; k < 4; ++k) s4[k] += (double)h[i * 4 + k];
    fprintf(stderr, "[conv_fast stamps] <%d,%d,%d,m%d,%d> %dx%d CinK %d CoutS %d wgs %zu | s_memtime ticks per wg: setup + first "
            "halo + LDS store %.0f, barrier %.0f, k-loops (all slabs) %.0f, epilogue %.0f\n", KC, TH, NT,
            mode == 1 ? 1 : (a.rows2 ? (a.H2 > 0 ? 3 : 2) : 0), NW, a.H, a.W, a.CinK, a.CoutS, nwg, s4[0] / nwg, s4[1] / nwg,
            s4[2] / nwg, s4[3] / nwg);
  }
}

bool launch_conv_fast(const ConvArgs& c, int th, hipStream_t st, bool dry) {
  if (c.H < th || c.W < 14) return false;
  if (c.in_mode == 2) {
    if (c.CinS != 1 || c.CoutS != 16 || th != 14) return false;
    FastArgs a;
    if (c.x2 != nullptr) return false;
    if (c.y_hi != nullptr) return false;
    if (c.x_up2) return false;
    a.x = (const unsigned char*)c.x; a.x2 = nullptr; a.y = (unsigned char*)c.y; a.y_hi = nullptr; a.wp = (const u32x4*)c.wp; a.stats = c.stats;
    a.up2 = 0;
    a.in_scale = a.in_shift = nullptr;
    a.y2 = nullptr; a.scale2 = a.shift2 = a.mean2 = nullptr; a.rows2 = nullptr; a.H2 = a.W2 = 0; a.img2 = nullptr;
    a.N = c.N; a.H = c.H; a.W = c.W; a.CinK = 16; a.CoutS = 16;
    static const int env_img_remap = lab_env("SPCL_IMAGE_XCD_REMAP", 1);
    a.tilesX = cdiv(c.W, 14); a.tilesY = cdiv(c.H, 14); a.gy = 1; a.xcd_remap = env_img_remap; a.lds_flip = 0; a.stamps = nullptr;
    a.acorr_rows = c.acorr_rows;
    a.stats_acc = a.rows2_acc = nullptr;
    a.in_bn = BnAccFwd{};
    if (c.stats_acc != nullptr || c.rows2_acc != nullptr || c.in_bn != nullptr) return false;
    if (c.acorr_rows != nullptr && !(c.H % 14 == 0 && c.W % 14 == 0)) return false;
    if (!dry) {
      if (c.acorr_rows != nullptr) SPCL_LAUNCH((conv3x3_image_kernel<14, true, true>), dim3(a.tilesX, a.tilesY, a.N), dim3(64), 0, st, a);
      else if (c.H % 14 == 0 && c.W % 14 == 0) SPCL_LAUNCH((conv3x3_image_kernel<14, true>), dim3(a.tilesX, a.tilesY, a.N), dim3(64), 0, st, a);
      else SPCL_LAUNCH((conv3x3_image_kernel<14, false>), dim3(a.tilesX, a.tilesY, a.N), dim3(64), 0, st, a);
    }
    return true;
  }
  if (c.CinS != c.CinK) return false;
  const bool wants_acc = c.stats_acc != nullptr || c.rows2_acc != nullptr || c.in_bn != nullptr;
  const int ntn = c.CoutS / 16, KC = conv_kc(c.CinK);
  static const int env_nt1 = lab_env("SPCL_CONV_FAST_NT1", 0);
  int NT = ntn >= 2 ? 2 : 1;
  if (env_nt1 == 1 && KC == 64 && ntn == 2) NT = 1;
  if (env_nt1 != 2 && KC == 64 && ntn == 2 && c.rows2 != nullptr && c.H2 > 0) NT = 1;
  if (env_nt1 != 2 && KC == 64 && ntn == 2) NT = 1;
  if (KC == 64 && ntn == 4 && env_nt1 != 3 && (c.in_mode == 1 || c.H <= 28)) NT = 1;
  static const int env_wide = lab_env("SPCL_CONV_FAST_NT1_WIDE", 1);
  if (env_wide && KC == 64 && ntn == 4 && c.CinK > 64) NT = 1;
  static const int env_all4 = lab_env("SPCL_CONV_FAST_NT1_64", 1);
  if (env_all4 && KC == 64 && ntn == 4) NT = 1;
  static const int env_fill = lab_env("SPCL_CONV_FAST_FILL", 1);
  static const int env_fill_max = lab_env("SPCL_CONV_FAST_FILL_MAX", 512);
  if (env_fill && KC == 64 && NT == 2 && ntn >= 8 && ntn % 4 == 0 &&
      (long)c.N * cdiv(c.W, 14) * cdiv(c.H, th) * cdiv(ntn, 8) < env_fill_max)
    NT = 1;
  static const int env_narrow = lab_env("SPCL_CONV_FAST_NARROW_NT1", 2);
  if (env_narrow == 1 && KC < 64 && ntn == 2 && th == 7) NT = 1;
  if (env_narrow == 2 && KC == 32 && ntn == 2 && th == 7 && c.rows2 != nullptr && c.H2 == 0 && c.img2 == nullptr) NT = 1;
  int nw = ntn / NT;
  if (nw > 4) nw = 4;
  if (ntn % (NT * nw) != 0) return false;
  FastArgs a;
  a.x = (const unsigned char*)c.x; a.y = (unsigned char*)c.y; a.wp = (const u32x4*)c.wp; a.stats = c.stats;
  a.x2 = (const unsigned char*)c.x2;
  a.y_hi = (unsigned char*)c.y_hi;
  a.up2 = c.x_up2 ? 1 : 0;
  if (c.x_up2 && !(c.in_mode == 0 && c.x2 == nullptr && c.rows2 == nullptr && c.img2 == nullptr && c.H % 2 == 0 &&
                   c.W % 2 == 0 && (double)c.N * c.H * c.W / 4.0 * c.CinK * 2.0 < 2147483648.0))
    return false;
  if (c.y_hi != nullptr && !(c.in_mode == 0 && (c.rows2 == nullptr || c.H2 == 0) && c.img2 == nullptr && c.stats == nullptr &&
                             ntn % 2 == 0))
    return false;
  if (c.x2 != nullptr && !(((c.CinK == KC && KC >= 32) || (KC == 64 && (c.CinK / 64) % 2 == 0)) && c.rows2 == nullptr &&
                           c.img2 == nullptr))
    return false;
  if (c.x2 != nullptr && c.in_mode == 1 && c.CinK != KC) return false;
  a.in_scale = c.in_scale; a.in_shift = c.in_shift;
  a.y2 = (const unsigned char*)c.y2; a.scale2 = c.scale2; a.shift2 = c.shift2; a.mean2 = c.mean2; a.rows2 = c.rows2;
  a.H2 = c.H2; a.W2 = c.W2;
  a.img2 = c.img2;
  a.acorr_rows = nullptr;
  a.stats_acc = c.stats_acc;
  a.rows2_acc = c.rows2_acc;
  a.in_bn = c.in_bn != nullptr ? *c.in_bn : BnAccFwd{};
  if (wants_acc) {
    const long tiles = (long)c.N * cdiv(c.W, 14) * cdiv(c.H, th);
    if (c.y_hi != nullptr || c.img2 != nullptr) return false;
    if (c.stats_acc != nullptr && (c.rows2 != nullptr || tiles > BN_ACC_MAX_TILES_FWD)) return false;
    if (c.rows2_acc != nullptr && (c.rows2 == nullptr || tiles > BN_ACC_MAX_TILES_BWD)) return false;
    if (c.in_bn != nullptr && !(c.in_mode == 1 && KC == 64 && c.x2 == nullptr && c.in_bn->CS == c.CinK &&
                                (c.CinK * 4 == 64 * nw || c.CinK * 2 == 64 * nw || c.CinK == 64 * nw)))
      return false;
  }
  if (c.rows2 != nullptr && c.in_mode != 0) return false;
  if (c.img2 != nullptr && !(c.rows2 != nullptr && c.H2 == 0 && KC == 16 && th == 14 && ntn == 1)) return false;
  a.N = c.N; a.H = c.H; a.W = c.W; a.CinK = c.CinK; a.CoutS = c.CoutS;
  a.tilesX = cdiv(c.W, 14); a.tilesY = cdiv(c.H, th); a.gy = ntn / (NT * nw);
  static const int env_remap = lab_env("SPCL_CONV_XCD_REMAP", 1);
  a.xcd_remap = (env_remap && a.gy == 1) ? 1 : 0;
  if (c.rows2 != nullptr && c.H2 > 0 && KC == 64 && nw == 1) return false;
#define SPCL_FAST_CASE(KC_, TH_, NT_, NW_)                               \
  if (KC == KC_ && th == TH_ && NT == NT_ && nw == NW_) {                \
    if (!dry) launch_fast<KC_, TH_, NT_, NW_>(a, c.in_mode, st);         \
    return true;                                                         \
  }
  SPCL_FAST_CASE(16, 14, 1, 1)
  SPCL_FAST_CASE(16, 14, 2, 1)
  SPCL_FAST_CASE(32, 14, 1, 1)
  SPCL_FAST_CASE(16, 7, 2, 1)
  SPCL_FAST_CASE(16, 7, 1, 2)
  SPCL_FAST_CASE(32, 7, 1, 2)
  SPCL_FAST_CASE(32, 7, 1, 1)
  SPCL_FAST_CASE(32, 7, 2, 1)
  SPCL_FAST_CASE(32, 7, 2, 2)
  SPCL_FAST_CASE(64, 7, 2, 1)
  SPCL_FAST_CASE(64, 7, 1, 2)
  SPCL_FAST_CASE(64, 7, 2, 2)
  SPCL_FAST_CASE(64, 7, 1, 4)
  SPCL_FAST_CASE(64, 7, 2, 4)
#undef SPCL_FAST_CASE
  return false;
}

}
```

self-paced-contrastive-learning_amd/functional.py:

```python
from __future__ import annotations

import ctypes
import os
from ctypes import c_double, c_float, c_int

import torch

from . import native as _n

SP_NONE, SP_HARD, SP_SOFT = 0, 1, 2


def take_grad_sink(param, needed: bool = True):
    if not needed or param is None:
        return None
    sink = getattr(param, "_grad_sink", None)
    if sink is None or not getattr(param, "_grad_sink_armed", False):
        return None
    if sink.shape != param.shape or sink.dtype != torch.float32 or not sink.is_contiguous() or sink.device != param.device:
        return None
    param._grad_sink_armed = False
    return sink


# ... 824 lines not shown
        sizes.append((_n.call("spcl_conv_packed_elems", ci, co, 0, dtc), _n.call("spcl_conv_packed_elems", ci, co, 1, dtc)))
    for i in range(0, len(layers), _n.PACK_MULTI_MAX):
        part, psz = layers[i:i + _n.PACK_MULTI_MAX], sizes[i:i + _n.PACK_MULTI_MAX]
        buf = torch.empty(sum(a + b for a, b in psz), dtype=dtype, device=dev)
        items, keep, off = [], [], 0
        for (w, H, W), (n0, n1) in zip(part, psz):
            wc = w.detach().contiguous().float()
            p0, p1 = buf[off:off + n0], buf[off + n0:off + n0 + n1]
            off += n0 + n1
            items.append(_n.PackItem(wc.data_ptr(), p0.data_ptr(), p1.data_ptr(), w.shape[1], w.shape[0],
                                     int(H) if _PACK_AT else 0, int(W) if _PACK_AT else 0))
            keep.append(wc)
            _PREPACKED[(w.data_ptr(), w._version, dtc, int(H), int(W))] = (p0, p1)
        arr = (_n.PackItem * len(items))(*items)
        if image is not None and i == 0 and _acorr_in_conv_rows(dtc, *[int(v) for v in image.shape[:3]]) > 0:
            image = None
        zero = _acc_arena_take_dirty(dev) if i == 0 else None
        zbytes = ctypes.c_size_t(zero.numel() * 8 if zero is not None else 0)
        if image is not None and i == 0:
            N, H, W = int(image.shape[0]), int(image.shape[1]), int(image.shape[2])
            acorr = torch.empty(_n.call("spcl_image_autocorr_rows", N, H, W), 64, dtype=torch.float32, device=dev)
            _n.call("spcl_conv_pack_weights_multi_zero", arr, len(items), dtc, _n.ptr(image), N, H, W, _n.ptr(acorr),
                    _n.ptr(zero), zbytes, _n.stream())
            _PREPACKED_ACORR[(image.data_ptr(), image._version)] = acorr
        else:
            _n.call("spcl_conv_pack_weights_multi_zero", arr, len(items), dtc, None, 0, 0, 0, None, _n.ptr(zero), zbytes,
                    _n.stream())


def _acorr_in_conv_rows(dt_code, N, H, W, cin=1, cout_s=16):
    return _n.call("spcl_conv3x3_forward_image_acorr_rows", dt_code, N, H, W, cin, cout_s)


def _conv_image_acorr(x_store, dt_code, dtype, N, H, W, cin_s, cout_s, wp, want_stats, rows):
    dev = x_store.device
    y = torch.empty(N, H, W, cout_s, dtype=dtype, device=dev)
    stats = None
    if want_stats:
        nt = _n.call("spcl_conv_stat_rows", dt_code, N, H, W, 16, cout_s)
        stats = torch.empty(_n.call("spcl_bn_stats_elems", nt, cout_s), dtype=torch.float32, device=dev)
        stats.ntiles = nt
    acorr = torch.empty(rows, 64, dtype=torch.float32, device=dev)
    _n.call("spcl_conv3x3_forward_image_acorr", _n.ptr(x_store), dt_code, N, H, W, cin_s, cout_s, _n.ptr(wp), _n.ptr(y),
            _n.ptr(stats), _n.ptr(acorr), _n.stream())
    return y, stats, acorr


def take_prepacked(w, dtc, H, W):
    return _PREPACKED.pop((w.data_ptr(), w._version, dtc, int(H), int(W)), None)


def _conv(x_store, dt_code, dtype, N, H, W, cin_s, cin_k, cout_s, wp, in_mode, scale, shift, want_stats):
    dev = x_store.device
    y = torch.empty(N, H, W, cout_s, dtype=dtype, device=dev)
    stats = None
    if want_stats:
        nt = _n.call("spcl_conv_stat_rows", dt_code, N, H, W, cin_k, cout_s)
        stats = torch.empty(_n.call("spcl_bn_stats_elems", nt, cout_s), dtype=torch.float32, device=dev)
        stats.ntiles = nt
    _n.call("spcl_conv3x3_forward", _n.ptr(x_store), dt_code, N, H, W, cin_s, cin_k, cout_s, _n.ptr(wp), in_mode,
            _n.ptr(scale), _n.ptr(shift), _n.ptr(y), _n.ptr(stats), _n.stream())
    return y, stats


def _conv_cat(xa, xb, dt_code, dtype, N, H, W, chalf, cout_s, wp, want_stats, xb_scale=None, xb_shift=None):
    dev = xa.device
    y = torch.empty(N, H, W, cout_s, dtype=dtype, device=dev)
    stats = None
    if want_stats:
        nt = _n.call("spcl_conv_stat_rows", dt_code, N, H, W, 2 * chalf, cout_s)
        stats = torch.empty(_n.call("spcl_bn_stats_elems", nt, cout_s), dtype=torch.float32, device=dev)
        stats.ntiles = nt
    _n.call("spcl_conv3x3_forward_cat", _n.ptr(xa), _n.ptr(xb), dt_code, N, H, W, chalf, cout_s, _n.ptr(wp),
            _n.ptr(xb_scale), _n.ptr(xb_shift), _n.ptr(y), _n.ptr(stats), _n.stream())
    return y, stats


_BN_ACC = os.environ.get("SPCL_BN_ACC", "1") != "0"
# ... 324 lines not shown
    return first, dgamma, dbeta


_IMAGE3 = os.environ.get("SPCL_IMAGE3", "1") != "0"


def _image3_supported(cfg, cin, dt_code, N, H, W, cout_s):
    return bool(_IMAGE3 and cfg.image_input and cin == 1 and cfg.dtype == torch.bfloat16 and W <= 256 and
                _n.call("spcl_conv_dgrad_bnstats_image_supported", dt_code, N, H, W, cout_s, cout_s))


def _image_autocorr(image, N, H, W):
    rows = _n.call("spcl_image_autocorr_rows", N, H, W)
    out = torch.empty(rows, 64, dtype=torch.float32, device=image.device)
    _n.call("spcl_image_autocorr", _n.ptr(image), N, H, W, _n.ptr(out), _n.stream())
    return out


def _dgrad_bnstats_image(dy, wp_t, y2, st2, image, dt_code, dtype, N, H, W, cs, want_g=False):
    dev = dy.device
    nt = _n.call("spcl_conv_stat_rows", dt_code, N, H, W, cs, cs)
    g = torch.empty(N, H, W, cs, dtype=dtype, device=dev) if want_g else None
    rows = torch.empty(nt * 11 * cs, dtype=torch.float32, device=dev)
    _n.call("spcl_conv3x3_dgrad_bnstats_image", _n.ptr(dy), dt_code, N, H, W, cs, cs, _n.ptr(wp_t), _n.ptr(g), _n.ptr(y2),
            _n.ptr(st2[2]), _n.ptr(st2[3]), _n.ptr(st2[0]), _n.ptr(image), _n.ptr(rows), _n.stream())
    rows.ntiles = nt
    return g, rows


_CONV16_FUSED = os.environ.get("SPCL_CONV16_FUSED", "1") != "0"
_CONV16_WGROWS = os.environ.get("SPCL_CONV16_WGROWS", "1") != "0"


def _conv16_bwd_fused(dy, wp_t, y2, st2, image, dt_code, N, H, W, cin, cout, cs, sink, acorr=None):
    dev = dy.device
    nsplit = _n.call("spcl_conv16_bwd_fused_splits", N, H, W)
    if acorr is not None:
        rows = torch.empty(11 * cs * nsplit, dtype=torch.float32, device=dev)
        rows.wg, rows.acorr16 = nsplit, torch.empty(16, 64, dtype=torch.float32, device=dev)
    else:
        nt = _n.call("spcl_conv_stat_rows", dt_code, N, H, W, cs, cs)
        rows = torch.empty(nt * 11 * cs, dtype=torch.float32, device=dev)
        rows.ntiles, rows.wg = nt, 0
    ws = torch.empty(nsplit * 9 * 256, dtype=torch.float32, device=dev)
    dw = _grad_buffer(sink, (cout, cin, 3, 3), dev)

    def launch():
        _n.call("spcl_conv16_bwd_fused", _n.ptr(dy), dt_code, N, H, W, _n.ptr(wp_t), _n.ptr(y2), _n.ptr(st2[2]),
                _n.ptr(st2[3]), _n.ptr(st2[0]), _n.ptr(image), _n.ptr(rows) if not rows.wg else None, _n.ptr(ws), _n.ptr(dw),
                cin, cout, _n.ptr(rows) if rows.wg else None, _n.ptr(acorr), 0 if acorr is None else acorr.shape[0],
                _n.ptr(rows.acorr16) if rows.wg else None, _n.stream())

    queue = sink_queue(sink)
    if queue is not None and _TAILS:
        if queue.capture_tail(sink, (ws, dy, y2, image, rows), launch):
            return None, rows
        return dw, rows
    launch()
    return dw, rows


def _bnrelu_bwd_rows_image3(rows, acorr, w, N, H, W, C, cs, st, training, sinks):
    dev = rows.device
    ws = torch.empty(_n.call("spcl_bnrelu_image3_workspace_bytes", cs) // 4, dtype=torch.float32, device=dev)
    dw = _grad_buffer(sinks[0], (C, 1, 3, 3), dev)
    dgamma, dbeta = _grad_buffer(sinks[1], (C,), dev), _grad_buffer(sinks[2], (C,), dev)
    wc = w.detach().contiguous().float()
    if getattr(rows, "wg", 0):
        _n.call("spcl_bnrelu_backward_wgrows_image3", _n.ptr(rows), rows.wg, _n.ptr(rows.acorr16), 16, _n.ptr(wc), N, H, W, C,
                cs, _n.ptr(st[0]), _n.ptr(st[1]), _n.ptr(st[2]), int(training), _n.ptr(ws), _n.ptr(dgamma), _n.ptr(dbeta),
                _n.ptr(dw), _n.stream())
        return dw, dgamma, dbeta
    _n.call("spcl_bnrelu_backward_rows_image3", _n.ptr(rows), rows.ntiles, _n.ptr(acorr), acorr.shape[0], _n.ptr(wc), N, H,
            W, C, cs, _n.ptr(st[0]), _n.ptr(st[1]), _n.ptr(st[2]), int(training), _n.ptr(ws), _n.ptr(dgamma), _n.ptr(dbeta),
            _n.ptr(dw), _n.stream())
    return dw, dgamma, dbeta


def _bnrelu_pool_bwd_rows(y, dpool, rows, dt_code, dtype, N, H, W, C, cs, st, training, sinks):
    dev = y.device
    ws = torch.empty(_n.call("spcl_bnrelu_bwd_workspace_bytes", N, H, W, cs) // 4, dtype=torch.float32, device=dev)
    dgamma = _grad_buffer(sinks[0], (C,), dev)
    dbeta = _grad_buffer(sinks[1], (C,), dev)
    dy = torch.empty(N, H, W, cs, dtype=dtype, device=dev)
    _n.call("spcl_bnrelu_pool_backward_rows", _n.ptr(y), _n.ptr(dpool), _n.ptr(rows), rows.ntiles, dt_code, N, H, W, C, cs,
            _n.ptr(st[0]), _n.ptr(st[1]), _n.ptr(st[2]), _n.ptr(st[3]), int(training), _n.ptr(ws), _n.ptr(dgamma),
            _n.ptr(dbeta), _n.ptr(dy), _n.stream())
    return dy, dgamma, dbeta
# ... 77 lines not shown
            xs = x.detach().float().permute(0, 2, 3, 1).contiguous()
            cin_s, cin_k, mode_a = cin, 16, 2
        else:
            xs = to_nhwc_padded(x.detach(), dtype)
            cin_s = cin_k = xs.shape[3]
            mode_a = 0
        need_bwd = any(ctx.needs_input_grad)
        ctx.acorr = None
        acorr_rows = 0
        if (need_bwd and ctx.needs_input_grad[1] and not ctx.needs_input_grad[0]
                and _image3_supported(cfg, cin, dtc, N, H, W, cout_s)):
            ctx.acorr = take_prepacked_acorr(xs)
            acorr_rows = _acorr_in_conv_rows(dtc, N, H, W, cin, cout_s) if (ctx.acorr is None and x2s is None) else 0
            if ctx.acorr is None and acorr_rows == 0:
                ctx.acorr = _image_autocorr(xs, N, H, W)
        pre_a, pre_b = take_prepacked(wa, dtc, H, W), take_prepacked(wb, dtc, H, W)
        if pre_a is not None and pre_b is not None:
            (wpa, wpa_t), (wpb, wpb_t) = pre_a, pre_b
        elif need_bwd:
            (wpa, wpa_t), (wpb, wpb_t) = _pack_block(wa, wb, dtc, dtype, *((H, W) if _PACK_AT else (0, 0)))
        else:
            wpa, wpb, wpa_t, wpb_t = _pack(wa, 0, dtc, dtype), _pack(wb, 0, dtc, dtype), None, None
        ctx.up2 = bool(getattr(cfg, "up2", False)) and cfg.need_act and not cfg.need_pool
        lazy = (bool(getattr(cfg, "lazy_act", False)) and cfg.need_act and not cfg.need_pool and not ctx.up2
                and getattr(cfg, "act_dst", None) is None)
        count = float(N) * H * W
        acc_ok = _BN_ACC and cfg.training and dtype == torch.bfloat16 and cout_s <= 256 and cout == cout_s
        sup = lambda ci, co, kind, out: bool(_n.call("spcl_conv_bn_acc_supported", dtc, N, H, W, ci, co, kind, out))
        use_a = (acc_ok and x2s is None and acorr_rows == 0 and mode_a == 0 and sup(cin_k, cout_s, 0, 1)
                 and sup(cout_s, cout_s, 1, 0))
        use_b = (acc_ok and not lazy and not ctx.up2 and getattr(cfg, "act_dst", None) is None
                 and sup(cout_s, cout_s, 1 if use_a else 2, 1))
        keep = []
        ctx.acc_bwd_a = ctx.acc_bwd_b = ctx.acc_rows_a = None
        if use_a:
            acc_a = bn_acc_block(cout_s, dev)
            ya, _ = _conv_acc(xs, dtc, dtype, N, H, W, cin_k, cout_s, wpa, None, None, None, acc_a, False)
            sta = torch.empty(4, cout_s, dtype=torch.float32, device=dev)
            bn_a = _bn_acc_desc(acc_a, cfg, cout, cout_s, ga, ba, 0, count, sta, keep)
        else:
            if x2s is not None:
                ya, sa = _conv_cat(xs, x2s, dtc, dtype, N, H, W, chalf, cout_s, wpa, cfg.training, *ctx.x2_coef)
            elif acorr_rows > 0:
                ya, sa, ctx.acorr = _conv_image_acorr(xs, dtc, dtype, N, H, W, cin_s, cout_s, wpa, cfg.training, acorr_rows)
            else:
                ya, sa = _conv(xs, dtc, dtype, N, H, W, cin_s, cin_k, cout_s, wpa, mode_a, None, None, cfg.training)
            sta = _bn_stats(sa, cfg, cout, cout_s, ga, ba, 0, dev)
        if use_a or use_b:
            acc_b = bn_acc_block(cout_s, dev) if use_b else None
            yb, sb = _conv_acc(ya, dtc, dtype, N, H, W, cout_s, cout_s, wpb, bn_a if use_a else None,
                               None if use_a else sta[2], None if use_a else sta[3], acc_b, cfg.training)
        else:
            yb, sb = _conv(ya, dtc, dtype, N, H, W, cout_s, cout_s, cout_s, wpb, 1, sta[2], sta[3], cfg.training)
        if use_b:
            stb = torch.empty(4, cout_s, dtype=torch.float32, device=dev)
            bn_b = _bn_acc_desc(acc_b, cfg, cout, cout_s, gb, bb, 1, count, stb, keep)
        else:
            stb = _bn_stats(sb, cfg, cout, cout_s, gb, bb, 1, dev)
        if acc_ok and any(ctx.needs_input_grad):
            if not cfg.image_input and _n.call("spcl_conv_dgrad_bnstats_acc_supported", dtc, N, H, W, cout_s, cout_s):
                ctx.acc_bwd_a = bn_acc_block(cout_s, dev)
            elif not cfg.image_input and _ACC_FILL:
                ctx.acc_rows_a = bn_acc_block(cout_s, dev)
            ctx.acc_bwd_b = bn_acc_block(cout_s, dev)
        cfg.gap = None
        want_gap = (_GAP and getattr(cfg, "want_gap", False) and cfg.need_act and not cfg.need_pool and not lazy
                    and not ctx.up2 and cfg.act_dst is None
                    and H * W <= 1024 and _n.call("spcl_bnrelu_gap_supported", dtc, H, W, cout, cout_s))
        if want_gap:
            act, pool = torch.empty(N, H, W, cout_s, dtype=dtype, device=dev), None
            cfg.gap = torch.empty(N, cout, dtype=torch.float32, device=dev)
            _n.call("spcl_bnrelu_gap_forward", _n.ptr(yb), dtc, N, H, W, cout, cout_s, None if use_b else _n.ptr(stb[2]),
                    None if use_b else _n.ptr(stb[3]), ctypes.byref(bn_b) if use_b else None, _n.ptr(act), _n.ptr(cfg.gap),
                    _n.stream())
        elif use_b:
            act = torch.empty(N, H, W, cout_s, dtype=dtype, device=dev) if cfg.need_act else None
            pool = torch.empty(N, H // 2, W // 2, cout_s, dtype=dtype, device=dev) if cfg.need_pool else None
            _n.call("spcl_bnrelu_pool_forward_acc", _n.ptr(yb), dtc, N, H, W, cout_s, ctypes.byref(bn_b), _n.ptr(act),
                    _n.ptr(pool), _n.stream())
        elif lazy:
            act, pool = yb, None
            cfg.link_act = ActLink(yb, stb, N, H, W, cout, cout_s)
        elif ctx.up2:
            act = torch.empty(N, 2 * H, 2 * W, cout_s, dtype=dtype, device=dev)
            pool = None
            _n.call("spcl_bnrelu_up2_forward", _n.ptr(yb), dtc, N, H, W, cout_s, _n.ptr(stb[2]), _n.ptr(stb[3]), _n.ptr(act),
# ... 74 lines not shown
                                                sk[4:6], acc)
            else:
                dyb, dgb, dbb = _bnrelu_bwd_bcast(yb, g_nc, dtc, dtype, N, H, W, cout, cout_s, stb, cfg.training, sk[4:6])
        elif lk is not None and da_s is None and dp_s is not None and lk.fresh(dp_s.data_ptr()):
            if lk.rows is ACC_ROWS:
                dyb, dgb, dbb = _bnrelu_bwd_acc(yb, None, dp_s, None, dtc, dtype, N, H, W, cout, cout_s, stb, cfg.training,
                                                sk[4:6], _take_acc(ctx, "acc_bwd_b"))
            else:
                acc = _take_acc(ctx, "acc_bwd_b") if (_ACC_FILL and H % 2 == 0 and W % 2 == 0 and cout_s <= 256) else None
                if acc is not None:
                    dyb, dgb, dbb = _bnrelu_bwd_rows_acc(yb, None, dp_s, lk.rows, dtc, dtype, N, H, W, cout, cout_s, stb,
                                                         cfg.training, sk[4:6], acc)
                else:
                    dyb, dgb, dbb = _bnrelu_pool_bwd_rows(yb, dp_s, lk.rows, dtc, dtype, N, H, W, cout, cout_s, stb,
                                                          cfg.training, sk[4:6])
        else:
            acc = _take_acc(ctx, "acc_bwd_b") if _ACC_FILL else None
            if acc is not None and lk is not None and lk.rows is ACC_ROWS:
                acc = None
            if acc is not None:
                dyb, dgb, dbb = _bnrelu_bwd_fill(yb, da_s, dp_s, dtc, dtype, N, H, W, cout, cout_s, stb, cfg.training, sk[4:6],
                                                 acc, dact_stride=da_stride, d_up=d_up)
            else:
                dyb, dgb, dbb = _bnrelu_bwd(yb, da_s, dp_s, dtc, dtype, N, H, W, cout, cout_s, stb, cfg.training, sk[4:6],
                                            dact_stride=da_stride, d_up=d_up)
        if lk is not None:
            lk.rows, lk.dx_ptr, lk.holder = None, 0, None
        if la is not None:
            la.rows, la.dx_ptr, la.holder = None, 0, None
        wpa_t, wpb_t = ctx.packed_t
        if wpb_t is None:
            wpb_t = _pack(wb, 1, dtc, dtype)
        image3 = ctx.acorr is not None
        one_pass = (image3 and _CONV16_FUSED and ctx.needs_input_grad[4] and cout == cout_s
                    and _n.call("spcl_conv16_bwd_fused_supported", dtc, N, H, W, cout_s, cout_s))
        if one_pass:
            dwb, rows16 = _conv16_bwd_fused(dyb, wpb_t, ya, sta, xs, dtc, N, H, W, cout, cout, cout_s, sk[3],
                                            acorr=ctx.acorr if _CONV16_WGROWS else None)
        else:
            dwb = _wgrad(ya, dyb, dtc, N, H, W, cout, cout_s, cout_s, cout, cout_s, 1, sta[2], sta[3], sk[3]) \
                if ctx.needs_input_grad[4] else None
        if one_pass:
            fused = (None, rows16)
        elif image3:
            fused = _dgrad_bnstats_image(dyb, wpb_t, ya, sta, xs, dtc, dtype, N, H, W, cout_s)
        else:
            acc = _take_acc(ctx, "acc_bwd_a")
            if acc is not None:
                fused = (_dgrad_bnstats_acc(dyb, wpb_t, ya, sta, dtc, dtype, N, H, W, cout_s, cout_s, acc), (ACC_ROWS, acc))
            else:
                fused = _dgrad_bnstats(dyb, wpb_t, ya, sta, dtc, dtype, N, H, W, cout_s, cout_s) \
                    if dtype == torch.bfloat16 else None
        if fused is not None:
            daa, rows = fused
        else:
            daa, _ = _conv(dyb, dtc, dtype, N, H, W, cout_s, cout_s, cout_s, wpb_t, 0, None, None, False)
        image_fused = ctx.needs_input_grad[1] and not ctx.needs_input_grad[0] and _image_wgrad_fusable(cfg, cin, cout_s)
        if image3:
            dya = None
            dwa, dga, dba = _bnrelu_bwd_rows_image3(rows, ctx.acorr, wa, N, H, W, cout, cout_s, sta, cfg.training, sk[0:3])
        elif image_fused:
            dya = None
            if fused is not None:
                dwa, dga, dba = _bnrelu_bwd_rows(ya, daa, xs, rows, dtc, dtype, N, H, W, cout, cout_s, sta, cfg.training,
                                                 sk[0:3])
            else:
                dwa, dga, dba = _bnrelu_bwd_image_wgrad(ya, daa, xs, dtc, N, H, W, cout, cout_s, sta, cfg.training,
                                                        sk[0:3])
        else:
            if fused is not None and isinstance(rows, tuple) and rows[0] is ACC_ROWS:
                dya, dga, dba = _bnrelu_bwd_acc(ya, daa, None, None, dtc, dtype, N, H, W, cout, cout_s, sta, cfg.training,
# ... 1268 lines not shown
```

self-paced-contrastive-learning_amd/native.py:

```python
from __future__ import annotations

import ctypes
import os
from ctypes import c_char_p, c_double, c_float, c_int, c_long, c_size_t, c_void_p

import torch

HERE = os.path.dirname(os.path.abspath(__file__))
LIB_PATH = os.path.join(HERE, "lib", "libspcl_hip.so")
SPCL_F32, SPCL_BF16 = 0, 1

_lib = None

_P = c_void_p
_SIGNATURES = {
    "spcl_abi_version": (c_int, []),
    "spcl_last_error": (c_char_p, []),
    "spcl_supcon_workspace_bytes": (c_size_t, [c_int, c_int]),
    "spcl_supcon_forward": (c_int, [_P, _P, _P, _P, c_int, c_int, c_float, c_int, c_float, c_int, _P, _P, _P]),
    "spcl_supcon_backward": (c_int, [_P, _P, c_int, c_int, c_float, c_int, c_float, _P, _P, _P, _P, _P, _P, _P]),
    "spcl_supcon_bwd_workspace_bytes": (c_size_t, [c_int, c_int]),
    "spcl_supcon_unit_gradient_block": (c_int, [c_int, c_int, _P, _P]),
    "spcl_supcon_materialize": (c_int, [_P, _P, c_int, c_int, c_float, c_int, c_float, _P, _P, _P, _P, _P, _P, _P]),
    "spcl_supcon_xpos_workspace_bytes": (c_size_t, [c_int, c_int]),
# ... 60 lines not shown
    "spcl_bn_eval_affine": (c_int, [c_int, c_int, _P, _P, _P, _P, c_float, _P, _P, _P, _P, _P]),
    "spcl_bn_eval_affine_multi": (c_int, [_P, c_int, _P]),
    "spcl_bnrelu_pool_forward": (c_int, [_P, c_int, c_int, c_int, c_int, c_int, _P, _P, _P, _P, _P]),
    "spcl_bnrelu_up2_forward": (c_int, [_P, c_int, c_int, c_int, c_int, c_int, _P, _P, _P, _P]),
    "spcl_bnrelu_pool_forward_strided": (c_int, [_P, c_int, c_int, c_int, c_int, c_int, _P, _P, _P, c_int, _P, _P]),
    "spcl_bnrelu_pool_backward_strided": (c_int, [_P, _P, c_int, _P, c_int, c_int, c_int, c_int, c_int, c_int, _P, _P, _P,
                                                  _P, c_int, _P, _P, _P, _P, _P]),
    "spcl_bnrelu_bwd_workspace_bytes": (c_size_t, [c_int, c_int, c_int, c_int]),
    "spcl_bnrelu_pool_backward": (c_int, [_P, _P, _P, c_int, c_int, c_int, c_int, c_int, c_int, _P, _P, _P, _P,
                                          c_int, _P, _P, _P, _P, _P]),
    "spcl_bnrelu_backward_up2": (c_int, [_P, _P, _P, c_int, c_int, c_int, c_int, c_int, c_int, _P, _P, _P, _P, c_int, _P, _P, _P, _P,
                                         _P]),
    "spcl_bnrelu_backward_bcast": (c_int, [_P, _P, c_int, c_int, c_int, c_int, c_int, c_int, _P, _P, _P, _P, c_int, _P, _P,
                                           _P, _P, _P]),
    "spcl_bnrelu_image_wgrad_workspace_bytes": (c_size_t, [c_int, c_int, c_int, c_int]),
    "spcl_bnrelu_backward_image_wgrad": (c_int, [_P, _P, _P, c_int, c_int, c_int, c_int, c_int, c_int, _P, _P, _P, _P,
                                                 c_int, _P, _P, _P, _P, _P]),
    "spcl_accumulate_scalars": (c_int, [c_int, _P, _P, _P, _P]),
    "spcl_stage_bytes": (c_int, [_P, _P, c_size_t, _P]),
    "spcl_conv_dgrad_bnstats_supported": (c_int, [c_int, c_int, c_int, c_int, c_int, c_int]),
    "spcl_conv3x3_dgrad_bnstats": (c_int, [_P, c_int, c_int, c_int, c_int, c_int, c_int, _P, _P, _P, _P, _P, _P, _P, _P]),
    "spcl_conv_dgrad_poolstats_supported": (c_int, [c_int, c_int, c_int, c_int, c_int, c_int, c_int, c_int]),
    "spcl_conv3x3_dgrad_poolstats": (c_int, [_P, c_int, c_int, c_int, c_int, c_int, c_int, _P, _P, _P, c_int, c_int, _P, _P,
                                             _P, _P, _P]),
    "spcl_bnrelu_pool_backward_rows": (c_int, [_P, _P, _P, c_int, c_int, c_int, c_int, c_int, c_int, c_int, _P, _P, _P, _P,
                                               c_int, _P, _P, _P, _P, _P]),
    "spcl_bnrelu_backward_rows": (c_int, [_P, _P, _P, _P, c_int, c_int, c_int, c_int, c_int, c_int, c_int, _P, _P, _P, _P,
                                          c_int, _P, _P, _P, _P, _P, _P]),
    "spcl_image_autocorr_rows": (c_int, [c_int, c_int, c_int]),
    "spcl_image_autocorr": (c_int, [_P, c_int, c_int, c_int, _P, _P]),
    "spcl_conv_dgrad_bnstats_image_supported": (c_int, [c_int, c_int, c_int, c_int, c_int, c_int]),
    "spcl_conv3x3_forward_image_acorr_rows": (c_int, [c_int, c_int, c_int, c_int, c_int, c_int]),
    "spcl_conv3x3_forward_image_acorr": (c_int, [_P, c_int, c_int, c_int, c_int, c_int, c_int, _P, _P, _P, _P, _P]),
    "spcl_conv16_bwd_fused_supported": (c_int, [c_int, c_int, c_int, c_int, c_int, c_int]),
    "spcl_conv16_bwd_fused_splits": (c_int, [c_int, c_int, c_int]),
    "spcl_conv16_bwd_fused": (c_int, [_P, c_int, c_int, c_int, c_int, _P, _P, _P, _P, _P, _P, _P, _P, _P, c_int, c_int,
                                      _P, _P, c_int, _P, _P]),
    "spcl_bnrelu_backward_wgrows_image3": (c_int, [_P, c_int, _P, c_int, _P, c_int, c_int, c_int, c_int, c_int, _P, _P, _P,
                                                   c_int, _P, _P, _P, _P, _P]),
    "spcl_conv3x3_dgrad_bnstats_image": (c_int, [_P, c_int, c_int, c_int, c_int, c_int, c_int, _P, _P, _P, _P, _P, _P, _P,
                                                 _P, _P]),
    "spcl_bnrelu_image3_workspace_bytes": (c_size_t, [c_int]),
    "spcl_bnrelu_backward_rows_image3": (c_int, [_P, c_int, _P, c_int, _P, c_int, c_int, c_int, c_int, c_int, _P, _P, _P,
                                                 c_int, _P, _P, _P, _P, _P]),
    "spcl_conv1x1_forward": (c_int, [_P, c_int, c_size_t, c_int, c_int, c_int, _P, _P, _P, _P]),
    "spcl_conv1x1_bwd_workspace_bytes": (c_size_t, [c_int, c_int]),
    "spcl_conv1x1_backward": (c_int, [_P, _P, c_int, c_size_t, c_int, c_int, c_int, _P, _P, _P, _P, _P, _P]),
    "spcl_conv1x1_forward_bn": (c_int, [_P, c_int, c_size_t, c_int, c_int, c_int, _P, _P, _P, _P, _P, _P]),
    "spcl_conv1x1_bwd_rows": (c_int, [c_size_t]),
    "spcl_conv1x1_backward_bn": (c_int, [_P, _P, c_int, c_size_t, c_int, c_int, c_int, _P, _P, _P, _P, _P, _P, _P, _P, _P, _P]),
    "spcl_softmax_forward": (c_int, [_P, c_size_t, c_int, _P, _P]),
    "spcl_softmax_backward": (c_int, [_P, _P, c_size_t, c_int, _P, _P]),
    "spcl_kl_workspace_bytes": (c_size_t, []),
    "spcl_kl_div_forward": (c_int, [_P, _P, c_size_t, c_int, c_float, _P, _P, _P]),
    "spcl_kl_div_backward": (c_int, [_P, _P, c_size_t, c_int, c_float, _P, _P, _P]),
    "spcl_sup_loss_forward": (c_int, [_P, _P, c_int, c_int, c_int, c_float, _P, _P, _P, _P, _P, _P]),
    "spcl_one_hot": (c_int, [_P, c_size_t, c_int, _P, _P]),
    "spcl_argmax_classes": (c_int, [_P, c_size_t, c_int, _P, _P]),
    "spcl_dice_counts": (c_int, [_P, _P, c_int, c_int, c_int, _P, _P, _P]),
    "spcl_surface_workspace_bytes": (c_size_t, [c_int, c_int, c_int, c_int]),
    "spcl_surface_distances": (c_int, [_P, _P, c_int, c_int, c_int, c_int, _P, c_int, c_double, c_double, c_double, _P, _P, _P,
                                       _P, _P, c_size_t, _P]),
    "spcl_surface_3d_workspace_bytes": (c_size_t, [c_int, c_int, c_int, c_int, c_int]),
    "spcl_surface_distances_3d": (c_int, [_P, _P, c_int, c_int, c_int, c_int, c_int, _P, c_int, c_double, c_double, c_double,
                                          c_double, _P, _P, _P, _P, _P, c_size_t, _P]),
    "spcl_upsample2x_forward": (c_int, [_P, _P, c_int, c_int, c_int, c_int, c_int, _P]),
# ... 91 lines not shown
class WgradItem(ctypes.Structure):
    _fields_ = [("x", c_void_p), ("dy", c_void_p), ("in_scale", c_void_p), ("in_shift", c_void_p),
                ("dw_oihw", c_void_p), ("N", c_int), ("H", c_int), ("W", c_int), ("Cin", c_int), ("CinS", c_int),
                ("Cout", c_int), ("CoutS", c_int), ("in_mode", c_int), ("x2", c_void_p), ("x_up2", c_int)]


class PackItem(ctypes.Structure):
    _fields_ = [("w_oihw", c_void_p), ("fwd", c_void_p), ("dgrad", c_void_p), ("Cin", c_int), ("Cout", c_int),
                ("H", c_int), ("W", c_int)]


BN_EVAL_MAX = 32


class BnEvalItem(ctypes.Structure):
    _fields_ = [("gamma", c_void_p), ("beta", c_void_p), ("running_mean", c_void_p), ("running_var", c_void_p),
                ("st", c_void_p), ("C", c_int), ("CS", c_int), ("eps", c_float)]


class BnAcc(ctypes.Structure):
    _fields_ = [("acc", c_void_p), ("gamma", c_void_p), ("beta", c_void_p), ("running_mean", c_void_p),
                ("running_var", c_void_p), ("num_batches_tracked", c_void_p), ("st", c_void_p), ("momentum", c_float),
                ("eps", c_float), ("count", c_float), ("C", c_int), ("CS", c_int)]


PACK_MULTI_MAX = 24


class WgradTail(ctypes.Structure):
    _fields_ = [("partial", c_void_p), ("dw", c_void_p), ("kind", c_int), ("nsplit", c_int), ("nblk_ci", c_int),
                ("nblk_co", c_int), ("CIB", c_int), ("COB", c_int), ("Cin", c_int), ("Cout", c_int)]


ABI_VERSION = 18
WGRAD_BATCH_MAX = 16
WGRAD_TAILS_MAX = 16
_NO_STATUS = ("spcl_abi_version", "spcl_conv3x3_forward_image_acorr_rows", "spcl_image_autocorr_rows", "spcl_conv_dgrad_bnstats_image_supported", "spcl_conv16_bwd_fused_supported", "spcl_conv16_bwd_fused_splits", "spcl_conv_num_tiles", "spcl_conv_stat_rows", "spcl_conv_set_gemm", "spcl_conv_set_f32_split", "spcl_conv_get_f32_split", "spcl_supcon_unit_gradient_block", "spcl_conv_cat_supported", "spcl_conv_up2_supported", "spcl_conv_split_supported", "spcl_conv_split_bnstats_supported", "spcl_conv1x1_bwd_rows", "spcl_profile_count", "spcl_conv_dgrad_bnstats_supported", "spcl_conv_dgrad_poolstats_supported",
              "spcl_conv_wgrad_batched_supported", "spcl_conv_bn_acc_supported", "spcl_conv_dgrad_bnstats_acc_supported",
              "spcl_conv_dgrad_poolstats_acc_supported", "spcl_supcon_rows_supported", "spcl_bnrelu_gap_supported")


class NativeLibraryError(RuntimeError):
    pass


def lib():
    global _lib
    if _lib is None:
        if not os.path.exists(LIB_PATH):
            raise NativeLibraryError(
                f"{LIB_PATH} is missing: build it with `python self-paced-contrastive-learning_amd/build.py` "
                "(there is no CPU / eager fallback for the hot path)")
        L = ctypes.CDLL(LIB_PATH)
        L.spcl_abi_version.restype, L.spcl_abi_version.argtypes = c_int, []
        have = L.spcl_abi_version()
        if have != ABI_VERSION:
            raise NativeLibraryError(
                f"{LIB_PATH} has C-ABI version {have}, this binding was written for {ABI_VERSION} (include/spcl_hip.h "
                "SPCL_ABI_VERSION): a stale build -- rebuild with `python self-paced-contrastive-learning_amd/build.py`")
        for name, (res, args) in _SIGNATURES.items():
            fn = getattr(L, name, None)
            if fn is None:
                continue
            fn.restype, fn.argtypes = res, args
        _lib = L
    return _lib


def call(name: str, *args):
    L = lib()
# ... 37 lines not shown
```

Baseline: 31880 slices/s.

## Recompute first image conv output instead of storing it in block 1

For the first UNet block (1->16 channels, bf16), the forward pass no longer writes the first conv's output to memory. The second conv and the fused conv16 backward kernel rebuild that output on the fly from the input image and the packed first-layer weights, using an extra MFMA per tile. This cuts the 16-channel activation write in forward and its read in backward, which are large at 224x224 resolution. In exchange it adds recompute arithmetic and register pressure in both kernels, and it only applies when the image-specific kernels support the shape.

```diff
diff --git a/include/spcl_hip.h b/include/spcl_hip.h
--- a/include/spcl_hip.h
+++ b/include/spcl_hip.h
@@ -14,7 +14,7 @@
 #define SPCL_ELAUNCH (-2)
 #define SPCL_EUNSUPPORTED (-3)
 
-#define SPCL_ABI_VERSION 18
+#define SPCL_ABI_VERSION 19
 int spcl_abi_version(void);
 const char* spcl_last_error(void);
 
@@ -109,6 +109,11 @@
 int spcl_conv3x3_forward_image_acorr_rows(int dtype, int N, int H, int W, int CinS, int CoutS);
 int spcl_conv3x3_forward_image_acorr(const void* x, int dtype, int N, int H, int W, int CinS, int CoutS,
                                      const void* w_packed, void* y, float* stats, float* acorr_rows, void* stream);
+int spcl_block1_recompute_supported(int dtype, int N, int H, int W, int CinS, int CoutS);
+int spcl_block1_kernels_take(int dtype, int N, int H, int W, int CinS, int CoutS);
+int spcl_conv3x3_forward_from_image(const float* image, const void* y_image, int dtype, int N, int H, int W, int CoutS,
+                                    const void* w_packed_image, const float* in_scale, const float* in_shift,
+                                    const void* w_packed, void* y, float* stats, void* stream);
 int spcl_conv_cat_supported(int dtype, int N, int H, int W, int Chalf, int CoutS);
 int spcl_conv3x3_forward_cat(const void* xa, const void* xb, int dtype, int N, int H, int W, int Chalf, int CoutS,
                              const void* w_packed, const float* xb_scale, const float* xb_shift, void* y, float* stats,
@@ -232,6 +237,11 @@
                           const float* scale2, const float* shift2, const float* mean2, const float* image,
                           float* rows11, float* partial, float* dw_oihw, int Cin, int Cout, float* wg_rows,
                           const float* acorr, int nacorr, float* acorr16, void* stream);
+int spcl_conv16_bwd_fused_image_supported(int dtype, int N, int H, int W, int CinK, int CoutS);
+int spcl_conv16_bwd_fused_image(const void* dy, int dtype, int N, int H, int W, const void* w_packed_dgrad,
+                                const void* w_packed_image, const float* scale2, const float* shift2, const float* mean2,
+                                const float* image, float* rows11, float* partial, float* dw_oihw, int Cin, int Cout,
+                                float* wg_rows, const float* acorr, int nacorr, float* acorr16, void* stream);
 int spcl_bnrelu_backward_wgrows_image3(const float* wg_rows, int nwg, const float* acorr, int nacorr, const float* w_oihw,
                                        int N, int H, int W, int C, int CS, const float* mean, const float* invstd,
                                        const float* scale, int training, float* ws, float* dgamma, float* dbeta,
diff --git a/self-paced-contrastive-learning_amd/csrc/conv.hip b/self-paced-contrastive-learning_amd/csrc/conv.hip
--- a/self-paced-contrastive-learning_amd/csrc/conv.hip
+++ b/self-paced-contrastive-learning_amd/csrc/conv.hip
@@ -1118,20 +1118,28 @@
   return N * cdiv(H, 14) * cdiv(W, 14);
 }
 
+static bool image_acorr_kernel_takes(ConvArgs& a, int dtype, int N, int H, int W, int CinS, int CoutS) {
+  if (image_acorr_args(a, dtype, N, H, W, CinS, CoutS)) return true;
+  if (!spcl_block1_kernels_take(dtype, N, H, W, CinS, CoutS)) return false;
+  a.N = N; a.H = H; a.W = W; a.CinS = CinS; a.CinK = 16; a.CoutS = CoutS; a.in_mode = 2;
+  a.tilesX = a.tilesY = 0; a.tpw = 1; a.dbg = 0;
+  return true;
+}
+
 extern "C" int spcl_conv3x3_forward_image_acorr(const void* x, int dtype, int N, int H, int W, int CinS, int CoutS,
                                                 const void* w_packed, void* y, float* stats, float* acorr_rows,
                                                 void* stream) {
-  SPCL_CHECK_ARG(x && y && w_packed && acorr_rows, "conv3x3_forward_image_acorr: null pointer");
+  SPCL_CHECK_ARG(x && w_packed && acorr_rows, "conv3x3_forward_image_acorr: null pointer");
   ConvArgs a;
   a.x = x; a.y = y; a.wp = w_packed; a.stats = stats; a.in_scale = a.in_shift = nullptr;
-  if (!image_acorr_args(a, dtype, N, H, W, CinS, CoutS)) {
-    set_error("conv3x3_forward_image_acorr: unsupported configuration (ask spcl_conv3x3_forward_image_acorr_rows)");
+  if (!image_acorr_kernel_takes(a, dtype, N, H, W, CinS, CoutS)) {
+    set_error("conv3x3_forward_image_acorr: unsupported configuration (bf16, one input channel, 16 outputs, whole 14 x 14 tiles)");
     return SPCL_EUNSUPPORTED;
   }
   a.acorr_rows = acorr_rows;
   {
     const double px = (double)N * H * W;
-    prof_cost(px * (4.0 + CoutS * 2.0) + 9.0 * 16 * CoutS * 2.0 + (double)N * cdiv(H, 14) * cdiv(W, 14) * 256.0,
+    prof_cost(px * (4.0 + (y != nullptr ? CoutS * 2.0 : 0.0)) + 9.0 * 16 * CoutS * 2.0 + (double)N * cdiv(H, 14) * cdiv(W, 14) * 256.0,
               2.0 * px * 9.0 * CinS * CoutS + 2.0 * px * 2.0 * 256.0);
   }
   if (!launch_conv_fast(a, 14, (hipStream_t)stream)) {
@@ -1139,6 +1147,60 @@
     return SPCL_EUNSUPPORTED;
   }
   SPCL_LAUNCH_CHECK("conv3x3_forward_image_acorr");
+  return SPCL_OK;
+}
+
+static bool from_image_args(ConvArgs& a, int dtype, int N, int H, int W, int CoutS) {
+  if (!spcl_block1_kernels_take(dtype, N, H, W, 1, CoutS)) return false;
+  a.N = N; a.H = H; a.W = W; a.CinS = 16; a.CinK = 16; a.CoutS = 16; a.in_mode = 1;
+  a.tilesX = a.tilesY = 0; a.tpw = 1; a.dbg = 0;
+  return true;
+}
+
+extern "C" int spcl_block1_kernels_take(int dtype, int N, int H, int W, int CinS, int CoutS) {
+  static const bool off = lab_env("SPCL_ACORR_IN_CONV", 1) == 0 || lab_env("SPCL_CONV_NO_FAST", 0) != 0;
+  if (off || dtype != SPCL_BF16 || N <= 0 || H < 14 || W < 14 || H % 14 || W % 14 || CinS != 1 || CoutS != 16) return 0;
+  return spcl_conv16_bwd_fused_image_supported(dtype, N, H, W, 16, 16);
+}
+
+extern "C" int spcl_block1_recompute_supported(int dtype, int N, int H, int W, int CinS, int CoutS) {
+  static const int no_fast = lab_env("SPCL_CONV_NO_FAST", 0);
+  if (no_fast || CinS != 1 || CoutS != 16) return 0;
+  if (spcl_conv3x3_forward_image_acorr_rows(dtype, N, H, W, CinS, CoutS) <= 0) return 0;
+  if (!spcl_conv16_bwd_fused_supported(dtype, N, H, W, 16, 16) || !spcl_conv16_bwd_fused_image_supported(dtype, N, H, W, 16, 16))
+    return 0;
+  ConvArgs a;
+  float dummy = 0.f;
+  a.x = nullptr; a.y = nullptr; a.wp = nullptr; a.stats = nullptr; a.in_scale = a.in_shift = nullptr;
+  if (!from_image_args(a, dtype, N, H, W, CoutS) || conv_use_gemm(16, 16, H, W)) return 0;
+  a.img1 = &dummy;
+  const TileCfg t = pick_tile_k(H, W, 16, 16);
+  return (t.tw == 14 && t.th == 14 && launch_conv_fast(a, 14, nullptr, true)) ? 1 : 0;
+}
+
+extern "C" int spcl_conv3x3_forward_from_image(const float* image, const void* y_image, int dtype, int N, int H, int W,
+                                               int CoutS, const void* w_packed_image, const float* in_scale,
+                                               const float* in_shift, const void* w_packed, void* y, float* stats,
+                                               void* stream) {
+  SPCL_CHECK_ARG((image && w_packed_image) || y_image, "conv3x3_forward_from_image: null pointer");
+  SPCL_CHECK_ARG(in_scale && in_shift && w_packed && y, "conv3x3_forward_from_image: null pointer");
+  ConvArgs a;
+  a.x = y_image; a.y = y; a.wp = w_packed; a.stats = stats; a.in_scale = in_scale; a.in_shift = in_shift;
+  if (!from_image_args(a, dtype, N, H, W, CoutS)) {
+    set_error("conv3x3_forward_from_image: unsupported configuration (bf16, 16 -> 16 channels, whole 14 x 14 tiles)");
+    return SPCL_EUNSUPPORTED;
+  }
+  if (y_image == nullptr) { a.img1 = image; a.wp1 = w_packed_image; }
+  {
+    const double px = (double)N * H * W;
+    prof_cost(px * ((y_image != nullptr ? 32.0 : 4.0) + 32.0) + 2.0 * 9.0 * 16 * 16 * 2.0,
+              2.0 * px * 9.0 * 16 * 16 + (y_image != nullptr ? 0.0 : 2.0 * px * 9.0 * 16));
+  }
+  if (!launch_conv_fast(a, 14, (hipStream_t)stream)) {
+    set_error("conv3x3_forward_from_image: no kernel for N=%d H=%d W=%d", N, H, W);
+    return SPCL_EUNSUPPORTED;
+  }
+  SPCL_LAUNCH_CHECK("conv3x3_forward_from_image");
   return SPCL_OK;
 }
 
diff --git a/self-paced-contrastive-learning_amd/csrc/conv16_bwd.hip b/self-paced-contrastive-learning_amd/csrc/conv16_bwd.hip
--- a/self-paced-contrastive-learning_amd/csrc/conv16_bwd.hip
+++ b/self-paced-contrastive-learning_amd/csrc/conv16_bwd.hip
@@ -9,6 +9,7 @@
   const unsigned char* dy;
   const u32x4* wp;
   const unsigned char* y2;
+  const u32x4* wp_img;
   const float* scale2;
   const float* shift2;
   const float* mean2;
@@ -435,8 +436,9 @@
 constexpr int R16_TAB = R16_TRASH + 32;
 constexpr int B16_LDS_ROWS = R16_TAB + 128;
 
-template <bool SHIFTED, bool WGROWS>
+template <bool SHIFTED, bool WGROWS, bool RECOMP = false>
 __global__ __launch_bounds__(128) __attribute__((amdgpu_waves_per_eu(r16_wpe(SHIFTED)))) void conv16_bwd_rows_kernel(Bwd16Args a) {
+  static_assert(!(RECOMP && SHIFTED), "y2 from the image: whole 14 x 14 tiles");
   constexpr int NW = 2;
   constexpr int TH = B16_TH, TW = B16_TW, HW_ = B16_HW, RP = R16_RP, PS = B16_PS;
   constexpr int NSTEPS = 5, NTHR = 64 * NW, ITER = 512 / NTHR, RPI = NTHR / 32;
@@ -504,8 +506,18 @@
 
   float imgv[256 / NTHR];
   u32x4 v[ITER];
-  uint2 ypre[MW];
+  uint2 ypre[RECOMP ? 1 : MW];
   constexpr int PPT = 256 / NTHR;
+  short wraw[3] = {0, 0, 0};
+  if (RECOMP) {
+    const int gq = min((t0 & 63) >> 4, 2);
+    const bf16_t* wq = (const bf16_t*)a.wp_img;
+#pragma unroll
+    for (int kx = 0; kx < 3; ++kx) {
+      const int tap = 3 * gq + kx;
+      wraw[kx] = (short)wq[(size_t)(((tap >> 1) * 64) + (2 * (tap & 1)) * 16 + (t0 & 15)) * 8];
+    }
+  }
   auto rsrc = [](const void* p) { return __builtin_amdgcn_make_buffer_rsrc((void*)p, 0, 0x7fffffff, 0x00020000); };
   constexpr int OOB = (int)0x80000000u;
   auto issue_img = [&](const int n) {
@@ -556,7 +568,14 @@
   if (n_first < a.N) {
     issue_img(n_first);
     issue_halo(n_first);
-    issue_y2(n_first);
+    if (!RECOMP) issue_y2(n_first);
+  }
+  uint2 wfp = {0u, 0u};
+  if (RECOMP) {
+    const bool real = ((t0 & 63) >> 4) < 3;
+    wfp.x = real ? ((uint32_t)(unsigned short)wraw[0] | ((uint32_t)(unsigned short)wraw[1] << 16)) : 0u;
+    wfp.y = real ? (uint32_t)(unsigned short)wraw[2] : 0u;
+    asm volatile("" : "+v"(wfp.x), "+v"(wfp.y));
   }
   __syncthreads();
   uint2 dzp[MW];
@@ -672,6 +691,8 @@
 
     f32x4 ssum = {0.f, 0.f, 0.f, 0.f}, ssq = {0.f, 0.f, 0.f, 0.f};
     const unsigned xaddr = (unsigned)(R16_XT + wave * B16_XT_ROW + r16 * PS + (((g + (r16 >> 2)) & 3) << 3));
+    const int pc = min(r16, TW - 1);
+    const unsigned yaddr = (unsigned)(R16_IM + (pc & 1) * 512 + ((g < 3 ? g : 0) + wave) * 32 + (pc & ~1) * 2);
     {
       const unsigned lb = (unsigned)(R16_DY + (wave * RP + r16) * PS);
       const unsigned offs[NSTEPS] = {tabA[0] + lb, tabA[1] + lb, tabA[2] + lb, tabA[3] + lb, tabB + lb};
@@ -684,8 +705,19 @@
           acc = mfma_chunk<bf16_t>(wall[s], xf, acc);
         }
         const bool keep_y = !shifted || wave + NW * j >= oy;
-        const float yv[4] = {__uint_as_float(ypre[j].x << 16), __uint_as_float(ypre[j].x & 0xffff0000u),
-                             __uint_as_float(ypre[j].y << 16), __uint_as_float(ypre[j].y & 0xffff0000u)};
+        uint2 yr;
+        if (RECOMP) {
+          const uint2 xv = {*(const uint32_t*)(lds + yaddr + j * (NW * 32)), *(const uint32_t*)(lds + yaddr + j * (NW * 32) + 4)};
+          const f32x4 y = __builtin_amdgcn_mfma_f32_16x16x16bf16_1k(__builtin_bit_cast(s16x4, wfp), __builtin_bit_cast(s16x4, xv),
+                                                                    (f32x4){0.f, 0.f, 0.f, 0.f}, 0, 0, 0);
+          const f32x2 ylo = {y[0], y[1]}, yhi = {y[2], y[3]};
+          yr.x = __builtin_bit_cast(uint32_t, __builtin_convertvector(ylo, bf16x2v));
+          yr.y = __builtin_bit_cast(uint32_t, __builtin_convertvector(yhi, bf16x2v));
+        } else {
+          yr = ypre[j];
+        }
+        const float yv[4] = {__uint_as_float(yr.x << 16), __uint_as_float(yr.x & 0xffff0000u),
+                             __uint_as_float(yr.y << 16), __uint_as_float(yr.y & 0xffff0000u)};
         const f32x2 glo = {acc[0], acc[1]}, ghi = {acc[2], acc[3]};
         const uint32_t g0 = __builtin_bit_cast(uint32_t, __builtin_convertvector(glo, bf16x2v));
         const uint32_t g1 = __builtin_bit_cast(uint32_t, __builtin_convertvector(ghi, bf16x2v));
@@ -727,7 +759,7 @@
     }
     if (!(it + 1 < a.ipw && n + 1 < a.N)) break;
     issue_halo(n + 1);
-    issue_y2(n + 1);
+    if (!RECOMP) issue_y2(n + 1);
     issue_img(n + 1);
     second_half(n);
   }
@@ -802,16 +834,23 @@
   return cdiv(H, B16_TH) * cdiv(W, B16_TW) * cdiv(N, ipw);
 }
 
-extern "C" int spcl_conv16_bwd_fused(const void* dy, int dtype, int N, int H, int W, const void* w_packed_dgrad,
-                                     const void* y2, const float* scale2, const float* shift2, const float* mean2,
-                                     const float* image, float* rows11, float* partial, float* dw_oihw, int Cin, int Cout,
-                                     float* wg_rows, const float* acorr, int nacorr, float* acorr16, void* stream) {
-  SPCL_CHECK_ARG(dy && w_packed_dgrad && y2 && scale2 && shift2 && mean2 && image && partial && dw_oihw,
+static int conv16_bwd_fused_impl(const void* dy, int dtype, int N, int H, int W, const void* w_packed_dgrad,
+                                 const void* y2, const void* w_packed_image, const float* scale2, const float* shift2,
+                                 const float* mean2, const float* image, float* rows11, float* partial, float* dw_oihw,
+                                 int Cin, int Cout, float* wg_rows, const float* acorr, int nacorr, float* acorr16,
+                                 void* stream) {
+  SPCL_CHECK_ARG(dy && w_packed_dgrad && (y2 || w_packed_image) && scale2 && shift2 && mean2 && image && partial && dw_oihw,
                  "conv16_bwd_fused: null pointer");
   SPCL_CHECK_ARG((rows11 != nullptr) != (wg_rows != nullptr), "conv16_bwd_fused: exactly one of rows11 / wg_rows");
   SPCL_CHECK_ARG(wg_rows == nullptr || (acorr && acorr16 && nacorr > 0), "conv16_bwd_fused: wg_rows comes with the autocorrelation rows");
   SPCL_CHECK_ARG(Cin > 0 && Cin <= 16 && Cout > 0 && Cout <= 16, "conv16_bwd_fused: channel counts");
-  if (!spcl_conv16_bwd_fused_supported(dtype, N, H, W, 16, 16)) {
+  if (y2 == nullptr) {
+    if (!spcl_block1_kernels_take(dtype, N, H, W, 1, 16)) {
+      set_error("conv16_bwd_fused_image: unsupported configuration (bf16, 16 -> 16 channels, H and W multiples of 14)");
+      return SPCL_EUNSUPPORTED;
+    }
+  } else if (!spcl_conv16_bwd_fused_supported(dtype, N, H, W, 16, 16) &&
+             !spcl_block1_kernels_take(dtype, N, H, W, 1, 16)) {
     set_error("conv16_bwd_fused: unsupported configuration (bf16, 16 -> 16 channels, 14 x 14 tiles)");
     return SPCL_EUNSUPPORTED;
   }
@@ -819,6 +858,7 @@
   spcl_wgrad_tail* tail = take_tail_capture();
   Bwd16Args a;
   a.dy = (const unsigned char*)dy; a.wp = (const u32x4*)w_packed_dgrad; a.y2 = (const unsigned char*)y2;
+  a.wp_img = (const u32x4*)w_packed_image;
   a.scale2 = scale2; a.shift2 = shift2; a.mean2 = mean2; a.img = image; a.rows11 = rows11; a.partial = partial;
   a.wg_rows = wg_rows; a.acorr_in = acorr; a.nacorr = nacorr; a.acorr_out = acorr16;
   a.N = N; a.H = H; a.W = W; a.tilesX = cdiv(W, B16_TW); a.tilesY = cdiv(H, B16_TH);
@@ -829,7 +869,7 @@
   const int nz = cdiv(N, a.ipw), nsplit = a.tilesX * a.tilesY * nz;
   a.nwg = nsplit;
   const double px = (double)N * H * W;
-  prof_cost(px * 32.0 * 2.0 + px * 4.0 + (double)nsplit * 9 * 256 * 4.0, 2.0 * px * 9.0 * 256 * 2.0 + 2.0 * px * 9.0 * 16);
+  prof_cost(px * 32.0 * (y2 != nullptr ? 2.0 : 1.0) + px * 4.0 + (double)nsplit * 9 * 256 * 4.0, 2.0 * px * 9.0 * 256 * 2.0 + 2.0 * px * 9.0 * 16);
   a.stamps = nullptr;
   const bool want_stamps = SPCL_CONV16_STAMPS_BUILD && lab_flag("SPCL_CONV16_STAMPS");
   const size_t nwg = (size_t)nsplit;
@@ -848,7 +888,10 @@
     else if (wgr) B16_LAUNCH(true, NW_, true);              \
     else B16_LAUNCH(true, NW_, false);                      \
   }
-  if (nw == 2 && conv16_bwd_rowmap()) {
+  if (y2 == nullptr) {
+    if (wgr) SPCL_LAUNCH((conv16_bwd_rows_kernel<false, true, true>), grid, dim3(128), B16_LDS_ROWS, st, a);
+    else SPCL_LAUNCH((conv16_bwd_rows_kernel<false, false, true>), grid, dim3(128), B16_LDS_ROWS, st, a);
+  } else if (nw == 2 && conv16_bwd_rowmap()) {
 #define B16_ROWS(SH_, WG_) SPCL_LAUNCH((conv16_bwd_rows_kernel<SH_, WG_>), grid, dim3(128), B16_LDS_ROWS, st, a)
     if (even && wgr) B16_ROWS(false, true);
     else if (even) B16_ROWS(false, false);
@@ -857,7 +900,7 @@
 #undef B16_ROWS
   }
 #if SPCL_LAB
-  else {
+  else if (y2 != nullptr) {
     B16_CASE(1) B16_CASE(2) B16_CASE(4)
   }
 #endif
@@ -885,3 +928,28 @@
   SPCL_LAUNCH_CHECK("conv16_bwd_fused");
   return SPCL_OK;
 }
+
+extern "C" int spcl_conv16_bwd_fused(const void* dy, int dtype, int N, int H, int W, const void* w_packed_dgrad,
+                                     const void* y2, const float* scale2, const float* shift2, const float* mean2,
+                                     const float* image, float* rows11, float* partial, float* dw_oihw, int Cin, int Cout,
+                                     float* wg_rows, const float* acorr, int nacorr, float* acorr16, void* stream) {
+  SPCL_CHECK_ARG(y2 != nullptr, "conv16_bwd_fused: null pointer");
+  return conv16_bwd_fused_impl(dy, dtype, N, H, W, w_packed_dgrad, y2, nullptr, scale2, shift2, mean2, image, rows11, partial,
+                               dw_oihw, Cin, Cout, wg_rows, acorr, nacorr, acorr16, stream);
+}
+
+extern "C" int spcl_conv16_bwd_fused_image_supported(int dtype, int N, int H, int W, int CinK, int CoutS) {
+  return (dtype == SPCL_BF16 && CinK == 16 && CoutS == 16 && N > 0 && H >= B16_TH && W >= B16_TW && H % B16_TH == 0 &&
+          W % B16_TW == 0 && conv16_bwd_nw() == 2 && conv16_bwd_rowmap() && (double)H * W * 32.0 < 2147483648.0)
+             ? 1 : 0;
+}
+
+extern "C" int spcl_conv16_bwd_fused_image(const void* dy, int dtype, int N, int H, int W, const void* w_packed_dgrad,
+                                           const void* w_packed_image, const float* scale2, const float* shift2,
+                                           const float* mean2, const float* image, float* rows11, float* partial,
+                                           float* dw_oihw, int Cin, int Cout, float* wg_rows, const float* acorr, int nacorr,
+                                           float* acorr16, void* stream) {
+  SPCL_CHECK_ARG(w_packed_image != nullptr, "conv16_bwd_fused_image: null pointer");
+  return conv16_bwd_fused_impl(dy, dtype, N, H, W, w_packed_dgrad, nullptr, w_packed_image, scale2, shift2, mean2, image, rows11,
+                               partial, dw_oihw, Cin, Cout, wg_rows, acorr, nacorr, acorr16, stream);
+}
diff --git a/self-paced-contrastive-learning_amd/csrc/conv_common.hpp b/self-paced-contrastive-learning_amd/csrc/conv_common.hpp
--- a/self-paced-contrastive-learning_amd/csrc/conv_common.hpp
+++ b/self-paced-contrastive-learning_amd/csrc/conv_common.hpp
@@ -47,6 +47,8 @@
   void* y_hi = nullptr;
   bool x_up2 = false;
   float* acorr_rows = nullptr;
+  const float* img1 = nullptr;
+  const void* wp1 = nullptr;
   long long* stats_acc = nullptr;
   long long* rows2_acc = nullptr;
   const struct BnAccFwd* in_bn = nullptr;
diff --git a/self-paced-contrastive-learning_amd/csrc/conv_fast.hip b/self-paced-contrastive-learning_amd/csrc/conv_fast.hip
--- a/self-paced-contrastive-learning_amd/csrc/conv_fast.hip
+++ b/self-paced-contrastive-learning_amd/csrc/conv_fast.hip
@@ -18,6 +18,7 @@
   const float* in_shift;
   int N, H, W, CinK, CoutS, tilesX, tilesY, gy;
   unsigned long long* stamps;
+  int ipw;
   int lds_flip;
   int xcd_remap;
   const unsigned char* y2;
@@ -27,6 +28,8 @@
   float* rows2;
   int H2, W2;
   const float* img2;
+  const float* img1;
+  const u32x4* wp1;
   float* acorr_rows;
   long long* stats_acc;
   long long* rows2_acc;
@@ -72,7 +75,7 @@
   int w = (wgs * NW + 3) / 4;
   w = w > 4 ? 4 : (w < 1 ? 1 : w);
   const int acc = (SPCL_FAST_ROWMAP ? TH : (TH * 14 + 15) / 16) * NT * 4;
-  if (KC == 16 && MODE >= 2 && SPCL_FAST_YPRE_MINKC <= 16 && w > 3 && acc <= 80) return 3;
+  if (KC == 16 && MODE >= 2 && MODE <= 4 && SPCL_FAST_YPRE_MINKC <= 16 && w > 3 && acc <= 80) return 3;
   if (acc > 80 && w > 2) return 2;
   if (KC == 64 && NT == 1 && NW == 4 && w > 2) return SPCL_FAST_WPE_NT1_NW4;
   if (KC == 64 && NT == 1 && NW >= 2 && w > 2) return SPCL_FAST_WPE_NT1;
@@ -133,7 +136,9 @@
   const int gps = (KC < 64 ? KC : a.CinK) * 2;
 
   constexpr bool M2 = MODE == 2 || MODE == 4;
-  constexpr bool M1 = MODE == 1 || MODE >= 5;
+  constexpr bool M1 = MODE == 1 || (MODE >= 5 && MODE <= 7);
+  constexpr bool M8 = MODE == 8;
+  static_assert(!M8 || (KC == 16 && TH == 14 && NT == 1 && NW == 1), "MODE 8: the 16 -> 16 layer on 14 x 14 tiles, one wave");
   constexpr int ACC_TPC = MODE == 5 ? 4 : (MODE == 6 ? 2 : 1);
   float imgv[MODE == 4 ? 4 : 1];
   if (MODE == 4) {
@@ -192,10 +197,15 @@
   const size_t wstep = (size_t)ntn * 1024;
   u32x4 v[ITER];
   float ssc[8], ssh[8];
+  constexpr int IW8 = 18;
+  float imv8[M8 ? 6 : 1];
+  s16x4 wfrag8 = {0, 0, 0, 0};
+  f32x4 sc8 = {0.f, 0.f, 0.f, 0.f}, sh8 = {0.f, 0.f, 0.f, 0.f};
+  const int ir8 = lane / IW8, ic8 = lane - ir8 * IW8;
   constexpr bool STREAM_W = PRELOAD_SLAB && KC == 64;
   constexpr int WR = STREAM_W ? (NT == 1 ? SPCL_FAST_WR_NT1 : 9) : (PRELOAD_SLAB ? NSTEPS : 1);
   u32x4 wsl[WR][NT];
-  constexpr bool acc_in = MODE >= 5;
+  constexpr bool acc_in = MODE >= 5 && MODE <= 7;
   float* const coef_l = (float*)(lds + fast_lds_bytes(KC, TH) * (a.lds_flip != 0 ? 2 : 1));
   auto load_coef_lds = [&](int slab) {
     const int cc = two_chunks ? ch1 : ch;
@@ -265,7 +275,60 @@
         if (in_range) *(u32x4*)(lpw + (dky * RP + dkx) * PS) = tv;
       }
     };
-    if (M1 && !interior) stage(std::false_type{});
+    if constexpr (M8) {
+      typedef uint32_t __attribute__((may_alias)) pair_t;
+      typedef unsigned short __attribute__((may_alias)) half_t;
+      const pair_t* const pairs = (const pair_t*)lds;
+      half_t* const halves = (half_t*)lds;
+      unsigned short pb8[6];
+#pragma unroll
+      for (int k = 0; k < 6; ++k) {
+        const f32x2 pv = {imv8[k], 0.f};
+        pb8[k] = (unsigned short)__builtin_bit_cast(uint32_t, __builtin_convertvector(pv, bf16x2v));
+      }
+      if (lane < 3 * IW8) {
+#pragma unroll
+        for (int k = 0; k < 6; ++k) halves[2 * ((ir8 + 3 * k) * IW8 + ic8)] = pb8[k];
+        if (ic8 > 0) {
+#pragma unroll
+          for (int k = 0; k < 6; ++k) halves[2 * ((ir8 + 3 * k) * IW8 + ic8) - 1] = pb8[k];
+        }
+        if (ic8 == IW8 - 1) {
+#pragma unroll
+          for (int k = 0; k < 6; ++k) halves[2 * ((ir8 + 3 * k) * IW8 + ic8) + 1] = 0;
+        }
+      }
+      __syncthreads();
+      const int gx = x0 - 1 + r16;
+      const bool colin = gx >= 0 && gx < a.W;
+      const int gg = g < 3 ? g : 0;
+      uint2 hv[HW_];
+#pragma unroll
+      for (int hy = 0; hy < TH + 2; ++hy) {
+        const pair_t* src = pairs + (hy + gg) * IW8 + r16;
+        const uint2 xv = {src[0], src[2]};
+        const f32x4 y = __builtin_amdgcn_mfma_f32_16x16x16bf16_1k(wfrag8, __builtin_bit_cast(s16x4, xv),
+                                                                  (f32x4){0.f, 0.f, 0.f, 0.f}, 0, 0, 0);
+        const f32x2 ylo = {y[0], y[1]}, yhi = {y[2], y[3]};
+        const uint32_t p0 = __builtin_bit_cast(uint32_t, __builtin_convertvector(ylo, bf16x2v));
+        const uint32_t p1 = __builtin_bit_cast(uint32_t, __builtin_convertvector(yhi, bf16x2v));
+        const u32x4 raw = {p0, p1, 0u, 0u};
+        const float s4[8] = {sc8[0], sc8[1], sc8[2], sc8[3], 0.f, 0.f, 0.f, 0.f};
+        const float b4[8] = {sh8[0], sh8[1], sh8[2], sh8[3], 0.f, 0.f, 0.f, 0.f};
+        const u32x4 tv = bnrelu_regs<bf16_t>(raw, s4, b4);
+        hv[hy] = (uint2){tv[0], tv[1]};
+      }
+      if (!interior) {
+#pragma unroll
+        for (int hy = 0; hy < TH + 2; ++hy) {
+          const int gy = y0 - 1 + hy;
+          if (!(colin && gy >= 0 && gy < a.H)) hv[hy] = (uint2){0u, 0u};
+        }
+      }
+      __syncthreads();
+#pragma unroll
+      for (int hy = 0; hy < TH + 2; ++hy) *(uint2*)(lds + (hy * RP + r16) * PS + g * 8) = hv[hy];
+    } else if (M1 && !interior) stage(std::false_type{});
     else stage(std::true_type{});
     if (refill) issue_halo(slab + 1);
     if (stamp && slab == 0) t_store = __builtin_amdgcn_s_memtime();
@@ -338,7 +401,31 @@
     accp.load(a.in_bn.acc, a.CinK, acc_c, acc_has ? ACC_RPT * acc_part : 0);
     accprm.load(a.in_bn, acc_c);
   }
-  issue_halo(0, true);
+  if constexpr (M8) {
+    const float* im = a.img1 + (size_t)n * a.H * a.W;
+    const int gx = x0 - 2 + ic8;
+    const bool colok = gx >= 0 && gx < a.W;
+    const int gxc = gx < 0 ? 0 : (gx >= a.W ? a.W - 1 : gx);
+#pragma unroll
+    for (int k = 0; k < 6; ++k) {
+      const int gy = y0 - 2 + ir8 + 3 * k;
+      const int gyc = gy < 0 ? 0 : (gy >= a.H ? a.H - 1 : gy);
+      const float raw = im[(size_t)gyc * a.W + gxc];
+      imv8[k] = (colok && gy >= 0 && gy < a.H) ? raw : 0.f;
+    }
+    if (g < 3) {
+      const bf16_t* wq = (const bf16_t*)a.wp1;
+#pragma unroll
+      for (int kx = 0; kx < 3; ++kx) {
+        const int tap = 3 * g + kx;
+        wfrag8[kx] = (short)wq[(size_t)(((tap >> 1) * 64) + (2 * (tap & 1)) * 16 + r16) * 8];
+      }
+    }
+    sc8 = *(const f32x4*)(a.in_scale + 4 * g);
+    sh8 = *(const f32x4*)(a.in_shift + 4 * g);
+  } else {
+    issue_halo(0, true);
+  }
   if (PRELOAD_SLAB) {
 #pragma unroll
     for (int s = 0; s < WR; ++s)
@@ -668,7 +755,7 @@
   }
 }
 
-template <int TH, bool EVEN, bool ACORR = false>
+template <int TH, bool EVEN, bool ACORR = false, bool STORE = true>
 __global__ __launch_bounds__(64) __attribute__((amdgpu_waves_per_eu(4))) void conv3x3_image_kernel(FastArgs a) {
   constexpr int TW = 14, HW_ = 16, LW = HW_ + 2;
   constexpr bool RM = SPCL_FAST_ROWMAP != 0;
@@ -676,7 +763,8 @@
   __shared__ uint32_t pairs[(TH + 2) * LW];
   const int lane = threadIdx.x, r16 = lane & 15, g = lane >> 4;
   int tx = blockIdx.x, ty = blockIdx.y;
-  const int n = blockIdx.z;
+  const int n_first = STORE ? (int)blockIdx.z : (int)blockIdx.z * a.ipw;
+  const int n_end = STORE ? n_first + 1 : min(n_first + a.ipw, a.N);
   {
     const int T = a.tilesX * a.tilesY;
     if (a.xcd_remap && (T & 7) == 0) {
@@ -688,7 +776,6 @@
   }
   const int y0 = min(ty * TH, a.H - TH), x0 = min(tx * TW, a.W - TW);
   const int oy = ty * TH - y0, ox = tx * TW - x0;
-  const int tile = (n * a.tilesY + ty) * a.tilesX + tx;
 
   s16x4 wfrag = {0, 0, 0, 0};
   if (g < 3) {
@@ -700,134 +787,150 @@
     }
   }
 
-  const float* img = (const float*)a.x + (size_t)n * a.H * a.W;
-  {
-    const int hx = r16, gx = x0 - 1 + hx;
-    const bool colok = gx >= 0 && gx < a.W;
-    const int gxc = gx < 0 ? 0 : (gx >= a.W ? a.W - 1 : gx);
-#pragma unroll
-    for (int k = 0; k < (NHALO + 63) / 64; ++k) {
-      const int hy = g + 4 * k;
-      const int gy = y0 - 1 + hy;
+  constexpr int NK = (NHALO + 63) / 64;
+  const int gx = x0 - 1 + r16;
+  const bool colok = gx >= 0 && gx < a.W;
+  const int gxc = gx < 0 ? 0 : (gx >= a.W ? a.W - 1 : gx);
+  float raw[NK];
+  auto request = [&](const int n) {
+    const float* img = (const float*)a.x + (size_t)n * a.H * a.W;
+#pragma unroll
+    for (int k = 0; k < NK; ++k) {
+      const int gy = y0 - 1 + g + 4 * k;
       const int gyc = gy < 0 ? 0 : (gy >= a.H ? a.H - 1 : gy);
-      const float raw = img[(size_t)gyc * a.W + gxc];
-      const float v0 = (colok && gy >= 0 && gy < a.H) ? raw : 0.f;
-      float v1 = __shfl_down(v0, 1, 64);
-      if (hx == HW_ - 1) v1 = 0.f;
-      const f32x2 pv = {v0, v1};
-      if (NHALO % 64 == 0 || hy < TH + 2) pairs[hy * LW + hx] = __builtin_bit_cast(uint32_t, __builtin_convertvector(pv, bf16x2v));
-    }
-  }
-  if (lane < 2 * (TH + 2)) pairs[(lane >> 1) * LW + HW_ + (lane & 1)] = 0u;
-  __syncthreads();
-
-  f32x4 acc[MT];
-#pragma unroll
-  for (int i = 0; i < MT; ++i) {
-    int p = 16 * i + r16;
-    if (p >= NPIX) p = 0;
-    const int py = RM ? i : p / TW, px = RM ? r16 : p - py * TW;
-    const int gg = g < 3 ? g : 0;
-    const uint32_t* src = pairs + (py + gg) * LW + px;
-    const uint32_t lo = src[0], hi = src[2];
-    const uint2 xv = {lo, hi};
-    acc[i] = __builtin_amdgcn_mfma_f32_16x16x16bf16_1k(wfrag, __builtin_bit_cast(s16x4, xv),
-                                                       (f32x4){0.f, 0.f, 0.f, 0.f}, 0, 0, 0);
-  }
-
-  constexpr int DPY = RM ? 1 : 16 / TW, DPX = RM ? 0 : 16 % TW;
-  const int rowb = a.CoutS * 2;
-  unsigned char* yb = a.y + (((size_t)n * a.H + y0) * a.W + x0) * rowb + 4 * g * 2;
-  int py = RM ? 0 : r16 / TW, px = r16 - py * TW;
-  int ob = (py * a.W + px) * rowb;
-  const int dob = (DPY * a.W + DPX) * rowb, wrapo = (a.W - TW) * rowb;
-  f32x4 ssum = {0.f, 0.f, 0.f, 0.f}, ssq = {0.f, 0.f, 0.f, 0.f};
-  const bool shifted = !EVEN && (oy | ox) != 0;
-  int pyc = py;
-  uint2 pk[MT];
-  int obs[MT];
-  if (!RM || r16 < TW) {
-#pragma unroll
-  for (int i = 0; i < MT; ++i) {
-    const bool ok = RM || (16 * i + 15 < NPIX) || (16 * i + r16 < NPIX);
-    obs[i] = ob;
+      raw[k] = img[(size_t)gyc * a.W + gxc];
+    }
+  };
+  request(n_first);
+#pragma unroll 1
+  for (int n = n_first; n < n_end; ++n) {
+    const int tile = (n * a.tilesY + ty) * a.tilesX + tx;
+    if (!STORE && n > n_first) __syncthreads();
     {
-      const f32x2 lo = {acc[i][0], acc[i][1]}, hi = {acc[i][2], acc[i][3]};
-      pk[i].x = __builtin_bit_cast(uint32_t, __builtin_convertvector(lo, bf16x2v));
-      pk[i].y = __builtin_bit_cast(uint32_t, __builtin_convertvector(hi, bf16x2v));
-    }
-    if (ok) {
-      if (EVEN) {
-        ssum += acc[i];
-        ssq += acc[i] * acc[i];
-      } else {
-        const float keep = (!shifted || (pyc >= oy && px >= ox)) ? 1.f : 0.f;
-        const f32x4 av = acc[i] * keep;
-        ssum += av;
-        ssq += av * acc[i];
-      }
-    }
-    px += DPX;
-    pyc += DPY;
-    ob += dob;
-    if (!RM && px >= TW) {
-      px -= TW;
-      pyc += 1;
-      ob += wrapo;
-    }
-  }
-  constexpr int NPAIR = SPCL_FAST_WIDE_STORES ? (RM ? MT / 2 : (NPIX / 16) / 2) : 0;
-#pragma unroll
-  for (int p = 0; p < NPAIR; ++p) {
-    const int i = 2 * p;
-    const auto rx = __builtin_amdgcn_permlane16_swap(pk[i].x, pk[i + 1].x, false, false);
-    const auto ry = __builtin_amdgcn_permlane16_swap(pk[i].y, pk[i + 1].y, false, false);
-    const u32x4 v = {rx[0], ry[0], rx[1], ry[1]};
-    *(u32x4*)(yb + ((g & 1) ? obs[i + 1] - 8 : obs[i])) = v;
-  }
-#pragma unroll
-  for (int i = 2 * NPAIR; i < MT; ++i) {
-    const bool ok = RM || (16 * i + 15 < NPIX) || (16 * i + r16 < NPIX);
-    if (ok) *(uint2*)(yb + obs[i]) = pk[i];
-  }
-  }
-  if (a.stats != nullptr)
-    write_tile_stats(a.stats, tile, a.CoutS, 4 * g, r16, (float)((TH - oy) * (TW - ox)), ssum, ssq);
-  if (ACORR) {
-    static_assert(!ACORR || (EVEN && TH % 2 == 0), "autocorrelation rows: whole 14 x 14 tiles");
-    __shared__ float dsum[2][16][16];
-    const int tap = r16 < 9 ? r16 : 0, ky = tap / 3, kx = tap - 3 * ky;
-    const uint32_t* src = pairs + ((g >> 1) + ky) * LW + 8 * (g & 1) + kx;
-    const bool upper = (g & 1) != 0;
-    const u32x4 ones = {0x3f803f80u, 0x3f803f80u, 0x3f803f80u, 0x3f803f80u};
-    f32x4 D = {0.f, 0.f, 0.f, 0.f}, S = {0.f, 0.f, 0.f, 0.f};
-#pragma unroll
-    for (int ks = 0; ks < TH / 2; ++ks) {
-      const uint32_t* q = src + ks * 2 * LW;
-      const u32x4 fb = {q[0], q[2], q[4], q[6]};
-      u32x4 fa = fb;
-      fa[3] = upper ? 0u : fb[3];
-      D = __builtin_amdgcn_mfma_f32_16x16x32_bf16(__builtin_bit_cast(bf16x8, fa), __builtin_bit_cast(bf16x8, fb), D, 0, 0, 0);
-      S = __builtin_amdgcn_mfma_f32_16x16x32_bf16(__builtin_bit_cast(bf16x8, fa), __builtin_bit_cast(bf16x8, ones), S, 0, 0, 0);
-    }
-#pragma unroll
-    for (int r = 0; r < 4; ++r) {
-      dsum[0][4 * g + r][r16] = D[r];
-      dsum[1][4 * g + r][r16] = S[r];
-    }
+      const int hx = r16;
+#pragma unroll
+      for (int k = 0; k < NK; ++k) {
+        const int hy = g + 4 * k;
+        const int gy = y0 - 1 + hy;
+        const float v0 = (colok && gy >= 0 && gy < a.H) ? raw[k] : 0.f;
+        float v1 = __shfl_down(v0, 1, 64);
+        if (hx == HW_ - 1) v1 = 0.f;
+        const f32x2 pv = {v0, v1};
+        if (NHALO % 64 == 0 || hy < TH + 2) pairs[hy * LW + hx] = __builtin_bit_cast(uint32_t, __builtin_convertvector(pv, bf16x2v));
+      }
+    }
+    if (!STORE && n + 1 < n_end) request(n + 1);
+    if (lane < 2 * (TH + 2)) pairs[(lane >> 1) * LW + HW_ + (lane & 1)] = 0u;
     __syncthreads();
-    const int k = lane;
-    float v = 0.f;
-    if (k < 45) {
-      int ra = 0;
-#pragma unroll
-      for (int i = 1; i < 9; ++i) ra += k >= i * 9 - i * (i - 1) / 2 ? 1 : 0;
-      const int cb = ra + (k - (ra * 9 - ra * (ra - 1) / 2));
-      v = dsum[0][ra][cb];
-    } else if (k < 54) {
-      v = dsum[1][k - 45][0];
-    }
-    a.acorr_rows[(size_t)tile * 64 + k] = v;
+
+    f32x4 acc[MT];
+#pragma unroll
+    for (int i = 0; i < MT; ++i) {
+      int p = 16 * i + r16;
+      if (p >= NPIX) p = 0;
+      const int py = RM ? i : p / TW, px = RM ? r16 : p - py * TW;
+      const int gg = g < 3 ? g : 0;
+      const uint32_t* src = pairs + (py + gg) * LW + px;
+      const uint32_t lo = src[0], hi = src[2];
+      const uint2 xv = {lo, hi};
+      acc[i] = __builtin_amdgcn_mfma_f32_16x16x16bf16_1k(wfrag, __builtin_bit_cast(s16x4, xv),
+                                                         (f32x4){0.f, 0.f, 0.f, 0.f}, 0, 0, 0);
+    }
+
+    constexpr int DPY = RM ? 1 : 16 / TW, DPX = RM ? 0 : 16 % TW;
+    const int rowb = a.CoutS * 2;
+    unsigned char* yb = a.y + (((size_t)n * a.H + y0) * a.W + x0) * rowb + 4 * g * 2;
+    int py = RM ? 0 : r16 / TW, px = r16 - py * TW;
+    int ob = (py * a.W + px) * rowb;
+    const int dob = (DPY * a.W + DPX) * rowb, wrapo = (a.W - TW) * rowb;
+    f32x4 ssum = {0.f, 0.f, 0.f, 0.f}, ssq = {0.f, 0.f, 0.f, 0.f};
+    const bool shifted = !EVEN && (oy | ox) != 0;
+    int pyc = py;
+    uint2 pk[MT];
+    int obs[MT];
+    if (!RM || r16 < TW) {
+#pragma unroll
+    for (int i = 0; i < MT; ++i) {
+      const bool ok = RM || (16 * i + 15 < NPIX) || (16 * i + r16 < NPIX);
+      if (STORE) {
+        obs[i] = ob;
+        const f32x2 lo = {acc[i][0], acc[i][1]}, hi = {acc[i][2], acc[i][3]};
+        pk[i].x = __builtin_bit_cast(uint32_t, __builtin_convertvector(lo, bf16x2v));
+        pk[i].y = __builtin_bit_cast(uint32_t, __builtin_convertvector(hi, bf16x2v));
+      }
+      if (ok) {
+        if (EVEN) {
+          ssum += acc[i];
+          ssq += acc[i] * acc[i];
+        } else {
+          const float keep = (!shifted || (pyc >= oy && px >= ox)) ? 1.f : 0.f;
+          const f32x4 av = acc[i] * keep;
+          ssum += av;
+          ssq += av * acc[i];
+        }
+      }
+      px += DPX;
+      pyc += DPY;
+      ob += dob;
+      if (!RM && px >= TW) {
+        px -= TW;
+        pyc += 1;
+        ob += wrapo;
+      }
+    }
+    constexpr int NPAIR = !STORE ? 0 : (SPCL_FAST_WIDE_STORES ? (RM ? MT / 2 : (NPIX / 16) / 2) : 0);
+#pragma unroll
+    for (int p = 0; p < NPAIR; ++p) {
+      const int i = 2 * p;
+      const auto rx = __builtin_amdgcn_permlane16_swap(pk[i].x, pk[i + 1].x, false, false);
+      const auto ry = __builtin_amdgcn_permlane16_swap(pk[i].y, pk[i + 1].y, false, false);
+      const u32x4 v = {rx[0], ry[0], rx[1], ry[1]};
+      *(u32x4*)(yb + ((g & 1) ? obs[i + 1] - 8 : obs[i])) = v;
+    }
+#pragma unroll
+    for (int i = 2 * NPAIR; i < MT; ++i) {
+      const bool ok = RM || (16 * i + 15 < NPIX) || (16 * i + r16 < NPIX);
+      if (STORE && ok) *(uint2*)(yb + obs[i]) = pk[i];
+    }
+    }
+    if (a.stats != nullptr)
+      write_tile_stats(a.stats, tile, a.CoutS, 4 * g, r16, (float)((TH - oy) * (TW - ox)), ssum, ssq);
+    if (ACORR) {
+      static_assert(!ACORR || (EVEN && TH % 2 == 0), "autocorrelation rows: whole 14 x 14 tiles");
+      __shared__ float dsum[2][16][16];
+      const int tap = r16 < 9 ? r16 : 0, ky = tap / 3, kx = tap - 3 * ky;
+      const uint32_t* src = pairs + ((g >> 1) + ky) * LW + 8 * (g & 1) + kx;
+      const bool upper = (g & 1) != 0;
+      const u32x4 ones = {0x3f803f80u, 0x3f803f80u, 0x3f803f80u, 0x3f803f80u};
+      f32x4 D = {0.f, 0.f, 0.f, 0.f}, S = {0.f, 0.f, 0.f, 0.f};
+#pragma unroll
+      for (int ks = 0; ks < TH / 2; ++ks) {
+        const uint32_t* q = src + ks * 2 * LW;
+        const u32x4 fb = {q[0], q[2], q[4], q[6]};
+        u32x4 fa = fb;
+        fa[3] = upper ? 0u : fb[3];
+        D = __builtin_amdgcn_mfma_f32_16x16x32_bf16(__builtin_bit_cast(bf16x8, fa), __builtin_bit_cast(bf16x8, fb), D, 0, 0, 0);
+        S = __builtin_amdgcn_mfma_f32_16x16x32_bf16(__builtin_bit_cast(bf16x8, fa), __builtin_bit_cast(bf16x8, ones), S, 0, 0, 0);
+      }
+#pragma unroll
+      for (int r = 0; r < 4; ++r) {
+        dsum[0][4 * g + r][r16] = D[r];
+        dsum[1][4 * g + r][r16] = S[r];
+      }
+      __syncthreads();
+      const int k = lane;
+      float v = 0.f;
+      if (k < 45) {
+        int ra = 0;
+#pragma unroll
+        for (int i = 1; i < 9; ++i) ra += k >= i * 9 - i * (i - 1) / 2 ? 1 : 0;
+        const int cb = ra + (k - (ra * 9 - ra * (ra - 1) / 2));
+        v = dsum[0][ra][cb];
+      } else if (k < 54) {
+        v = dsum[1][k - 45][0];
+      }
+      a.acorr_rows[(size_t)tile * 64 + k] = v;
+    }
   }
 }
 
@@ -853,6 +956,9 @@
   if (a.img2 != nullptr) {
     if constexpr (KC == 16 && TH == 14 && NT == 1 && NW == 1)
       SPCL_LAUNCH((conv3x3_fast_kernel<KC, TH, NT, 4, NW>), grid, block, lds, st, b);
+  } else if (mode == 8) {
+    if constexpr (KC == 16 && TH == 14 && NT == 1 && NW == 1)
+      SPCL_LAUNCH((conv3x3_fast_kernel<KC, TH, NT, 8, NW>), grid, block, lds, st, b);
   } else if (mode == 1 && a.in_bn.acc != nullptr) {
     if constexpr (KC == 64) {
       const int tpc = 64 * NW / a.CinK;
@@ -895,12 +1001,19 @@
     static const int env_img_remap = lab_env("SPCL_IMAGE_XCD_REMAP", 1);
     a.tilesX = cdiv(c.W, 14); a.tilesY = cdiv(c.H, 14); a.gy = 1; a.xcd_remap = env_img_remap; a.lds_flip = 0; a.stamps = nullptr;
     a.acorr_rows = c.acorr_rows;
+    a.img1 = nullptr; a.wp1 = nullptr; a.ipw = 1;
     a.stats_acc = a.rows2_acc = nullptr;
     a.in_bn = BnAccFwd{};
     if (c.stats_acc != nullptr || c.rows2_acc != nullptr || c.in_bn != nullptr) return false;
     if (c.acorr_rows != nullptr && !(c.H % 14 == 0 && c.W % 14 == 0)) return false;
+    if (c.y == nullptr && !dry && c.acorr_rows == nullptr) return false;
     if (!dry) {
-      if (c.acorr_rows != nullptr) SPCL_LAUNCH((conv3x3_image_kernel<14, true, true>), dim3(a.tilesX, a.tilesY, a.N), dim3(64), 0, st, a);
+      if (c.acorr_rows != nullptr && c.y == nullptr) {
+        a.ipw = (int)(((long)a.tilesX * a.tilesY * a.N + 4095) / 4096);
+        a.ipw = a.ipw < 1 ? 1 : (a.ipw > a.N ? a.N : a.ipw);
+        SPCL_LAUNCH((conv3x3_image_kernel<14, true, true, false>), dim3(a.tilesX, a.tilesY, cdiv(a.N, a.ipw)), dim3(64), 0, st, a);
+      }
+      else if (c.acorr_rows != nullptr) SPCL_LAUNCH((conv3x3_image_kernel<14, true, true>), dim3(a.tilesX, a.tilesY, a.N), dim3(64), 0, st, a);
       else if (c.H % 14 == 0 && c.W % 14 == 0) SPCL_LAUNCH((conv3x3_image_kernel<14, true>), dim3(a.tilesX, a.tilesY, a.N), dim3(64), 0, st, a);
       else SPCL_LAUNCH((conv3x3_image_kernel<14, false>), dim3(a.tilesX, a.tilesY, a.N), dim3(64), 0, st, a);
     }
@@ -950,6 +1063,11 @@
   a.H2 = c.H2; a.W2 = c.W2;
   a.img2 = c.img2;
   a.acorr_rows = nullptr;
+  a.img1 = c.img1; a.wp1 = (const u32x4*)c.wp1; a.ipw = 1;
+  if (c.img1 != nullptr && !(c.in_mode == 1 && KC == 16 && th == 14 && ntn == 1 && c.x2 == nullptr && c.y_hi == nullptr &&
+                             !c.x_up2 && c.rows2 == nullptr && c.img2 == nullptr && !wants_acc && c.H % 14 == 0 && c.W % 14 == 0 &&
+                             (dry || (c.wp1 != nullptr && c.in_scale != nullptr && c.in_shift != nullptr))))
+    return false;
   a.stats_acc = c.stats_acc;
   a.rows2_acc = c.rows2_acc;
   a.in_bn = c.in_bn != nullptr ? *c.in_bn : BnAccFwd{};
@@ -971,7 +1089,7 @@
   if (c.rows2 != nullptr && c.H2 > 0 && KC == 64 && nw == 1) return false;
 #define SPCL_FAST_CASE(KC_, TH_, NT_, NW_)                               \
   if (KC == KC_ && th == TH_ && NT == NT_ && nw == NW_) {                \
-    if (!dry) launch_fast<KC_, TH_, NT_, NW_>(a, c.in_mode, st);         \
+    if (!dry) launch_fast<KC_, TH_, NT_, NW_>(a, c.img1 != nullptr ? 8 : c.in_mode, st); \
     return true;                                                         \
   }
   SPCL_FAST_CASE(16, 14, 1, 1)
diff --git a/self-paced-contrastive-learning_amd/functional.py b/self-paced-contrastive-learning_amd/functional.py
--- a/self-paced-contrastive-learning_amd/functional.py
+++ b/self-paced-contrastive-learning_amd/functional.py
@@ -880,9 +880,9 @@
     return _n.call("spcl_conv3x3_forward_image_acorr_rows", dt_code, N, H, W, cin, cout_s)
 
 
-def _conv_image_acorr(x_store, dt_code, dtype, N, H, W, cin_s, cout_s, wp, want_stats, rows):
+def _conv_image_acorr(x_store, dt_code, dtype, N, H, W, cin_s, cout_s, wp, want_stats, rows, store=True):
     dev = x_store.device
-    y = torch.empty(N, H, W, cout_s, dtype=dtype, device=dev)
+    y = torch.empty(N, H, W, cout_s, dtype=dtype, device=dev) if store else None
     stats = None
     if want_stats:
         nt = _n.call("spcl_conv_stat_rows", dt_code, N, H, W, 16, cout_s)
@@ -892,6 +892,22 @@
     _n.call("spcl_conv3x3_forward_image_acorr", _n.ptr(x_store), dt_code, N, H, W, cin_s, cout_s, _n.ptr(wp), _n.ptr(y),
             _n.ptr(stats), _n.ptr(acorr), _n.stream())
     return y, stats, acorr
+
+
+_BLOCK1_RECOMPUTE = os.environ.get("SPCL_BLOCK1_RECOMPUTE", "1") != "0"
+
+
+def _conv_from_image(image, y_image, dt_code, dtype, N, H, W, cout_s, wp_image, scale, shift, wp, want_stats):
+    dev = image.device
+    y = torch.empty(N, H, W, cout_s, dtype=dtype, device=dev)
+    stats = None
+    if want_stats:
+        nt = N * (H // 14) * (W // 14)
+        stats = torch.empty(_n.call("spcl_bn_stats_elems", nt, cout_s), dtype=torch.float32, device=dev)
+        stats.ntiles = nt
+    _n.call("spcl_conv3x3_forward_from_image", _n.ptr(image), _n.ptr(y_image), dt_code, N, H, W, cout_s, _n.ptr(wp_image),
+            _n.ptr(scale), _n.ptr(shift), _n.ptr(wp), _n.ptr(y), _n.ptr(stats), _n.stream())
+    return y, stats
 
 
 def take_prepacked(w, dtc, H, W):
@@ -1282,8 +1298,10 @@
 _CONV16_WGROWS = os.environ.get("SPCL_CONV16_WGROWS", "1") != "0"
 
 
-def _conv16_bwd_fused(dy, wp_t, y2, st2, image, dt_code, N, H, W, cin, cout, cs, sink, acorr=None):
+def _conv16_bwd_fused(dy, wp_t, y2, st2, image, dt_code, N, H, W, cin, cout, cs, sink, acorr=None, wp_image=None):
     dev = dy.device
+    if y2 is None and wp_image is None:
+        raise RuntimeError("conv16 backward: neither the first convolution's output nor its packed weights")
     nsplit = _n.call("spcl_conv16_bwd_fused_splits", N, H, W)
     if acorr is not None:
         rows = torch.empty(11 * cs * nsplit, dtype=torch.float32, device=dev)
@@ -1296,14 +1314,15 @@
     dw = _grad_buffer(sink, (cout, cin, 3, 3), dev)
 
     def launch():
-        _n.call("spcl_conv16_bwd_fused", _n.ptr(dy), dt_code, N, H, W, _n.ptr(wp_t), _n.ptr(y2), _n.ptr(st2[2]),
+        _n.call("spcl_conv16_bwd_fused" if y2 is not None else "spcl_conv16_bwd_fused_image", _n.ptr(dy), dt_code, N, H, W,
+                _n.ptr(wp_t), _n.ptr(y2 if y2 is not None else wp_image), _n.ptr(st2[2]),
                 _n.ptr(st2[3]), _n.ptr(st2[0]), _n.ptr(image), _n.ptr(rows) if not rows.wg else None, _n.ptr(ws), _n.ptr(dw),
                 cin, cout, _n.ptr(rows) if rows.wg else None, _n.ptr(acorr), 0 if acorr is None else acorr.shape[0],
                 _n.ptr(rows.acorr16) if rows.wg else None, _n.stream())
 
     queue = sink_queue(sink)
     if queue is not None and _TAILS:
-        if queue.capture_tail(sink, (ws, dy, y2, image, rows), launch):
+        if queue.capture_tail(sink, (ws, dy, y2, image, rows, wp_image), launch):
             return None, rows
         return dw, rows
     launch()
@@ -1447,6 +1466,7 @@
         use_b = (acc_ok and not lazy and not ctx.up2 and getattr(cfg, "act_dst", None) is None
                  and sup(cout_s, cout_s, 1 if use_a else 2, 1))
         keep = []
+        recompute = False
         ctx.acc_bwd_a = ctx.acc_bwd_b = ctx.acc_rows_a = None
         if use_a:
             acc_a = bn_acc_block(cout_s, dev)
@@ -1457,7 +1477,11 @@
             if x2s is not None:
                 ya, sa = _conv_cat(xs, x2s, dtc, dtype, N, H, W, chalf, cout_s, wpa, cfg.training, *ctx.x2_coef)
             elif acorr_rows > 0:
-                ya, sa, ctx.acorr = _conv_image_acorr(xs, dtc, dtype, N, H, W, cin_s, cout_s, wpa, cfg.training, acorr_rows)
+                recompute = (_BLOCK1_RECOMPUTE and _CONV16_FUSED and cfg.training and not use_b and cin == 1
+                             and cout == cout_s and ctx.needs_input_grad[4]
+                             and bool(_n.call("spcl_block1_recompute_supported", dtc, N, H, W, cin_s, cout_s)))
+                ya, sa, ctx.acorr = _conv_image_acorr(xs, dtc, dtype, N, H, W, cin_s, cout_s, wpa, cfg.training, acorr_rows,
+                                                      store=not recompute)
             else:
                 ya, sa = _conv(xs, dtc, dtype, N, H, W, cin_s, cin_k, cout_s, wpa, mode_a, None, None, cfg.training)
             sta = _bn_stats(sa, cfg, cout, cout_s, ga, ba, 0, dev)
@@ -1465,8 +1489,11 @@
             acc_b = bn_acc_block(cout_s, dev) if use_b else None
             yb, sb = _conv_acc(ya, dtc, dtype, N, H, W, cout_s, cout_s, wpb, bn_a if use_a else None,
                                None if use_a else sta[2], None if use_a else sta[3], acc_b, cfg.training)
+        elif recompute:
+            yb, sb = _conv_from_image(xs, None, dtc, dtype, N, H, W, cout_s, wpa, sta[2], sta[3], wpb, cfg.training)
         else:
             yb, sb = _conv(ya, dtc, dtype, N, H, W, cout_s, cout_s, cout_s, wpb, 1, sta[2], sta[3], cfg.training)
+        ctx.wpa_fwd = wpa if recompute else None
         if use_b:
             stb = torch.empty(4, cout_s, dtype=torch.float32, device=dev)
             bn_b = _bn_acc_desc(acc_b, cfg, cout, cout_s, gb, bb, 1, count, stb, keep)
@@ -1607,11 +1634,14 @@
         if wpb_t is None:
             wpb_t = _pack(wb, 1, dtc, dtype)
         image3 = ctx.acorr is not None
-        one_pass = (image3 and _CONV16_FUSED and ctx.needs_input_grad[4] and cout == cout_s
+        one_pass = (image3 and (_CONV16_FUSED or ya is None) and ctx.needs_input_grad[4] and cout == cout_s
                     and _n.call("spcl_conv16_bwd_fused_supported", dtc, N, H, W, cout_s, cout_s))
+        if ya is None and not one_pass:
+            raise RuntimeError("image block backward: the first convolution's output was not stored and the one-pass kernel "
+                               "that forms it again is not available")
         if one_pass:
             dwb, rows16 = _conv16_bwd_fused(dyb, wpb_t, ya, sta, xs, dtc, N, H, W, cout, cout, cout_s, sk[3],
-                                            acorr=ctx.acorr if _CONV16_WGROWS else None)
+                                            acorr=ctx.acorr if _CONV16_WGROWS else None, wp_image=ctx.wpa_fwd)
         else:
             dwb = _wgrad(ya, dyb, dtc, N, H, W, cout, cout_s, cout_s, cout, cout_s, 1, sta[2], sta[3], sk[3]) \
                 if ctx.needs_input_grad[4] else None
diff --git a/self-paced-contrastive-learning_amd/native.py b/self-paced-contrastive-learning_amd/native.py
--- a/self-paced-contrastive-learning_amd/native.py
+++ b/self-paced-contrastive-learning_amd/native.py
@@ -116,6 +116,12 @@
     "spcl_conv_dgrad_bnstats_image_supported": (c_int, [c_int, c_int, c_int, c_int, c_int, c_int]),
     "spcl_conv3x3_forward_image_acorr_rows": (c_int, [c_int, c_int, c_int, c_int, c_int, c_int]),
     "spcl_conv3x3_forward_image_acorr": (c_int, [_P, c_int, c_int, c_int, c_int, c_int, c_int, _P, _P, _P, _P, _P]),
+    "spcl_block1_recompute_supported": (c_int, [c_int, c_int, c_int, c_int, c_int, c_int]),
+    "spcl_block1_kernels_take": (c_int, [c_int, c_int, c_int, c_int, c_int, c_int]),
+    "spcl_conv3x3_forward_from_image": (c_int, [_P, _P, c_int, c_int, c_int, c_int, c_int, _P, _P, _P, _P, _P, _P, _P]),
+    "spcl_conv16_bwd_fused_image_supported": (c_int, [c_int, c_int, c_int, c_int, c_int, c_int]),
+    "spcl_conv16_bwd_fused_image": (c_int, [_P, c_int, c_int, c_int, c_int, _P, _P, _P, _P, _P, _P, _P, _P, _P, c_int, c_int,
+                                            _P, _P, c_int, _P, _P]),
     "spcl_conv16_bwd_fused_supported": (c_int, [c_int, c_int, c_int, c_int, c_int, c_int]),
     "spcl_conv16_bwd_fused_splits": (c_int, [c_int, c_int, c_int]),
     "spcl_conv16_bwd_fused": (c_int, [_P, c_int, c_int, c_int, c_int, _P, _P, _P, _P, _P, _P, _P, _P, _P, c_int, c_int,
@@ -273,10 +279,10 @@
                 ("nblk_co", c_int), ("CIB", c_int), ("COB", c_int), ("Cin", c_int), ("Cout", c_int)]
 
 
-ABI_VERSION = 18
+ABI_VERSION = 19
 WGRAD_BATCH_MAX = 16
 WGRAD_TAILS_MAX = 16
-_NO_STATUS = ("spcl_abi_version", "spcl_conv3x3_forward_image_acorr_rows", "spcl_image_autocorr_rows", "spcl_conv_dgrad_bnstats_image_supported", "spcl_conv16_bwd_fused_supported", "spcl_conv16_bwd_fused_splits", "spcl_conv_num_tiles", "spcl_conv_stat_rows", "spcl_conv_set_gemm", "spcl_conv_set_f32_split", "spcl_conv_get_f32_split", "spcl_supcon_unit_gradient_block", "spcl_conv_cat_supported", "spcl_conv_up2_supported", "spcl_conv_split_supported", "spcl_conv_split_bnstats_supported", "spcl_conv1x1_bwd_rows", "spcl_profile_count", "spcl_conv_dgrad_bnstats_supported", "spcl_conv_dgrad_poolstats_supported",
+_NO_STATUS = ("spcl_abi_version", "spcl_block1_recompute_supported", "spcl_block1_kernels_take", "spcl_conv16_bwd_fused_image_supported", "spcl_conv3x3_forward_image_acorr_rows", "spcl_image_autocorr_rows", "spcl_conv_dgrad_bnstats_image_supported", "spcl_conv16_bwd_fused_supported", "spcl_conv16_bwd_fused_splits", "spcl_conv_num_tiles", "spcl_conv_stat_rows", "spcl_conv_set_gemm", "spcl_conv_set_f32_split", "spcl_conv_get_f32_split", "spcl_supcon_unit_gradient_block", "spcl_conv_cat_supported", "spcl_conv_up2_supported", "spcl_conv_split_supported", "spcl_conv_split_bnstats_supported", "spcl_conv1x1_bwd_rows", "spcl_profile_count", "spcl_conv_dgrad_bnstats_supported", "spcl_conv_dgrad_poolstats_supported",
               "spcl_conv_wgrad_batched_supported", "spcl_conv_bn_acc_supported", "spcl_conv_dgrad_bnstats_acc_supported",
               "spcl_conv_dgrad_poolstats_acc_supported", "spcl_supcon_rows_supported", "spcl_bnrelu_gap_supported")
 
```

New measurement: 32200 slices/s (median of 6 runs). 1.01x the previous value.
